# octavian-ganea/equidock_public

Hardware: NVIDIA H100
Metric: protein_pairs_per_sec_iegmn_fwd_kabsch (higher is better)
Workload: dtype f32

## Files before the change

### equidock_public_b200/csrc/node_mlp_tc.cu

```cuda
#include "tc_common.cuh"

namespace eqd {

#define NM_THREADS 256
#define NM_W5_SPLIT 34816
#define NM_W6_BASE 104448
#define NM_W6_SPLIT 8192
#define NM_W_BYTES 129024

struct NmConsts { float b5[64], ln_g[64], ln_b[64], b6[64]; };

#define NM_CHAINS 2
#define NM_SLOTS 3

struct NmSmem {
  unsigned char w[NM_W_BYTES];
  float stage[NM_CHAINS][NM_SLOTS][64 * 64];
  float c[256];
  unsigned long long w_bar;
};

#define NM_HLN_BYTES 512
static_assert(sizeof(NmSmem) + 128 + NM_HLN_BYTES <= 232448, "node MLP shared memory exceeds the sm_90 limit");

template <int P, bool HLN>
__global__ void __launch_bounds__(NM_CHAINS * 128, 1)
node_mlp_tc_kernel(int n_nodes, eqd_layer_params p, const __grid_constant__ NmConsts cst, const float* __restrict__ h_in,
                   const float* __restrict__ aggr, const float* __restrict__ mu, const float* __restrict__ h0,
                   float* __restrict__ h_out, eqd_layer_norms nm) {
  extern __shared__ __align__(128) unsigned char smem_raw[];
  NmSmem& S = *reinterpret_cast<NmSmem*>(smem_raw);
  float* hln = reinterpret_cast<float*>(smem_raw + sizeof(NmSmem));
  const int tid = threadIdx.x, wgi = tid >> 7, t = tid & 127, lane = t & 31;
  float (&ring)[NM_SLOTS][64 * 64] = S.stage[wgi];
  const int bar = 1 + wgi;
  const int ntiles = (n_nodes + 63) / 64, tstride = gridDim.x * NM_CHAINS, tile0 = blockIdx.x * NM_CHAINS + wgi;
  if (tid == 0) {
    mbar_init(&S.w_bar, 1);
    asm volatile("fence.mbarrier_init.release.cluster;" ::: "memory");
    mbar_expect_tx(&S.w_bar, NM_W_BYTES);
    bulk_g2s(S.w, p.w_node_tc, NM_W_BYTES, &S.w_bar);
  }
  for (int i = tid; i < 256; i += NM_CHAINS * 128) S.c[i] = reinterpret_cast<const float*>(&cst)[i];
  if (HLN && tid < 128) hln[tid] = tid < 64 ? nm.final_ln_g[tid] : nm.final_ln_b[tid - 64];
  __syncthreads();
  const unsigned w_saddr = smem_u32(S.w);
  const float slope = p.leaky_slope, sk = p.skip_weight_h, sk1 = 1.f - p.skip_weight_h;
  const int fr0 = (t >> 5) * 16 + (lane >> 2), fc = 2 * (lane & 3);

  auto issue = [&](int q) {
    const int tile = tile0 + (q >> 2) * tstride, pc = q & 3;
    if (tile < ntiles) {
      const float* src = pc == 0 ? h_in : pc == 1 ? aggr : pc == 2 ? mu : h0;
      stage_rows64(ring[q % NM_SLOTS], src, pc == 3 ? EQD_H0_PAD : EQD_HID, 0, (long)tile * 64, min(64, n_nodes - tile * 64), t);
    } else {
      cp_async_commit();
    }
  };
  int q = 0;
  for (int i = 0; i < NM_SLOTS - 1; ++i) issue(i);
  mbar_wait(&S.w_bar, 0);

  for (int tile = tile0; tile < ntiles; tile += tstride) {
    const int node0 = tile * 64, nvalid = min(64, n_nodes - node0);
    float2 x4[2];
#pragma unroll
    for (int hh = 0; hh < 2; ++hh) {
      const int row = fr0 + 8 * hh;
      x4[hh] = row < nvalid ? *reinterpret_cast<const float2*>(h0 + (long)(node0 + row) * EQD_H0_PAD + 64 + fc)
                            : make_float2(0.f, 0.f);
    }
    float acc[32], hs[32];
#pragma unroll
    for (int j = 0; j < 8; ++j) {
      const float2 bj = *reinterpret_cast<const float2*>(&S.c[8 * j + fc]);
#pragma unroll
      for (int hh = 0; hh < 2; ++hh) {
        acc[4 * j + 2 * hh] = bj.x;
        acc[4 * j + 2 * hh + 1] = bj.y;
      }
    }
#pragma unroll 1
    for (int pc = 0; pc < 4; ++pc, ++q) {
      cp_async_wait<NM_SLOTS - 2>();
      wg_barrier(bar);
      issue(q + NM_SLOTS - 1);
      float v[32];
      staged_rows_to_frag(ring[q % NM_SLOTS], t, v);
      if (pc == 0) {
#pragma unroll
        for (int i = 0; i < 32; ++i) hs[i] = v[i];
      }
      unsigned af[3][4][4];
      acc_to_a_split3<4, P>(v, af);
      float d[32];
      wg_gemm6_rs_issue<64, 4, 0, false, P>(d, af, [&](int sp, int kb) {
        return b_desc_ex(w_saddr + (4 * pc + kb) * 2048 + sp * NM_W5_SPLIT, 1024, 128); }, false);
      wg_mma_wait(d);
#pragma unroll
      for (int i = 0; i < 32; ++i) acc[i] = __fadd_rn(acc[i], d[i]);
    }
    {
      unsigned a4[3][1][4];
#pragma unroll
      for (int hh = 0; hh < 2; ++hh) split3_pair<P>(x4[hh].x, x4[hh].y, a4[0][0][hh], a4[1][0][hh], a4[2][0][hh]);
#pragma unroll
      for (int sp = 0; sp < 3; ++sp) a4[sp][0][2] = a4[sp][0][3] = 0u;
      float d[32];
      wg_gemm6_rs_issue<64, 1, 0, false, P>(d, a4, [&](int sp, int kb) {
        return b_desc_ex(w_saddr + 16 * 2048 + sp * NM_W5_SPLIT, 1024, 128); }, false);
      wg_mma_wait(d);
#pragma unroll
      for (int i = 0; i < 32; ++i) acc[i] = __fadd_rn(acc[i], d[i]);
    }
    unsigned af[3][4][4];
    {
      float (&v)[32] = acc;
#pragma unroll
      for (int i = 0; i < 32; ++i) v[i] = fmaxf(v[i], __fmul_rn(v[i], slope));
      float pv[32];
#pragma unroll
      for (int i = 0; i < 32; ++i) pv[i] = __shfl_xor_sync(0xffffffffu, v[i], 2);
      float msum[2], rstd[2];
#pragma unroll
      for (int h = 0; h < 2; ++h) {
        float mh[2], qh[2];
#pragma unroll
        for (int ch = 0; ch < 2; ++ch) {
          float s0 = 0.f, s1 = 0.f;
#pragma unroll
          for (int c4 = 0; c4 < 8; ++c4) {
            s0 = __fadd_rn(s0, chain_val(v, pv, h, ch, c4, 0));
            s1 = __fadd_rn(s1, chain_val(v, pv, h, ch, c4, 1));
          }
          const float sp = __fadd_rn(s0, s1);
          mh[ch] = __fmul_rn(__fadd_rn(sp, __shfl_xor_sync(0xffffffffu, sp, 1)), 1.f / 32.f);
          float q0 = 0.f, q1 = 0.f;
#pragma unroll
          for (int c4 = 0; c4 < 8; ++c4) {
            const float d0 = __fadd_rn(chain_val(v, pv, h, ch, c4, 0), -mh[ch]);
            const float d1 = __fadd_rn(chain_val(v, pv, h, ch, c4, 1), -mh[ch]);
            q0 = __fmaf_rn(d0, d0, q0);
            q1 = __fmaf_rn(d1, d1, q1);
          }
          const float qp = __fadd_rn(q0, q1);
          qh[ch] = __fadd_rn(qp, __shfl_xor_sync(0xffffffffu, qp, 1));
        }
        msum[h] = __fadd_rn(mh[0], mh[1]);
        const float dm = __fadd_rn(mh[0], -mh[1]);
        const float var = __fmaf_rn(__fmul_rn(dm, dm), 16.f, __fadd_rn(qh[0], qh[1]));
        rstd[h] = 1.f / sqrtf(__fmaf_rn(var, 1.f / 64.f, 1e-5f));
      }
#pragma unroll
      for (int j = 0; j < 8; ++j) {
        const float2 gj = *reinterpret_cast<const float2*>(&S.c[64 + 8 * j + fc]);
        const float2 bj = *reinterpret_cast<const float2*>(&S.c[128 + 8 * j + fc]);
#pragma unroll
        for (int h = 0; h < 2; ++h) {
          float& x0 = v[4 * j + 2 * h];
          float& x1 = v[4 * j + 2 * h + 1];
          x0 = __fmaf_rn(__fmul_rn(__fmaf_rn(msum[h], -0.5f, x0), rstd[h]), gj.x, bj.x);
          x1 = __fmaf_rn(__fmul_rn(__fmaf_rn(msum[h], -0.5f, x1), rstd[h]), gj.y, bj.y);
        }
      }
      acc_to_a_split3<4, P>(v, af);
    }
    {
      float d[32];
      wg_gemm6_rs_issue<64, 4, 0, false, P>(d, af, [&](int sp, int kb) {
        return b_desc_ex(w_saddr + NM_W6_BASE + sp * NM_W6_SPLIT + kb * 2048, 1024, 128); }, false);
      wg_mma_wait(d);
      if (HLN) {
#pragma unroll
        for (int j = 0; j < 8; ++j) {
          const float2 bj = *reinterpret_cast<const float2*>(&S.c[192 + 8 * j + fc]);
#pragma unroll
          for (int hh = 0; hh < 2; ++hh) {
            const int i = 4 * j + 2 * hh;
            d[i] = __fmaf_rn(__fadd_rn(d[i], bj.x), sk, __fmul_rn(hs[i], sk1));
            d[i + 1] = __fmaf_rn(__fadd_rn(d[i + 1], bj.y), sk, __fmul_rn(hs[i + 1], sk1));
          }
        }
        float mean[2], rstd[2];
        quad_ln_stats(d, mean, rstd);
        quad_ln_apply(d, mean, rstd, hln, hln + 64, fc);
#pragma unroll
        for (int hh = 0; hh < 2; ++hh) {
          const int row = fr0 + 8 * hh;
          if (row < nvalid) {
            float* o = h_out + (long)(node0 + row) * EQD_HID + fc;
#pragma unroll
            for (int j = 0; j < 8; ++j)
              *reinterpret_cast<float2*>(o + 8 * j) = make_float2(d[4 * j + 2 * hh], d[4 * j + 2 * hh + 1]);
          }
        }
      } else
#pragma unroll
      for (int hh = 0; hh < 2; ++hh) {
        const int row = fr0 + 8 * hh;
        if (row < nvalid) {
          float* o = h_out + (long)(node0 + row) * EQD_HID + fc;
#pragma unroll
          for (int j = 0; j < 8; ++j) {
            const float2 bj = *reinterpret_cast<const float2*>(&S.c[192 + 8 * j + fc]);
            const int i = 4 * j + 2 * hh;
            *reinterpret_cast<float2*>(o + 8 * j) =
                make_float2(__fmaf_rn(__fadd_rn(d[i], bj.x), sk, __fmul_rn(hs[i], sk1)),
                            __fmaf_rn(__fadd_rn(d[i + 1], bj.y), sk, __fmul_rn(hs[i + 1], sk1)));
          }
        }
      }
    }
  }
  cp_async_wait<0>();
}


#define NM0_W5_SPLIT 35840
#define NM0_W6_BASE 107520
#define NM0_W6_SPLIT 10240
#define NM0_W_BYTES 138240
#define NM0_A_SPLIT 20480
#define NM0_LD 84

struct Nm0Consts { float b5[80], ln_g[80], ln_b[80], b6[64]; };

struct Nm0Smem {
  unsigned char w[NM0_W_BYTES];
  unsigned char a[3 * NM0_A_SPLIT];
  float red[EQD_TM * 4];
  unsigned long long w_bar;
};

template <bool HLN>
__global__ void __launch_bounds__(NM_THREADS, 1)
node_mlp0_tc_kernel(int n_nodes, eqd_layer_params p, const __grid_constant__ Nm0Consts cst, const float* __restrict__ h0,
                    const float* __restrict__ aggr, const float* __restrict__ mu , float* __restrict__ h_out,
                    eqd_layer_norms nm) {
  extern __shared__ __align__(128) unsigned char smem_raw[];
  Nm0Smem& S = *reinterpret_cast<Nm0Smem*>(smem_raw);
  const int tid = threadIdx.x, q = tid, half = q >> 7, r = q & 127, wgi = tid >> 7;
  const int ntiles = (n_nodes + EQD_TM - 1) / EQD_TM;
  if (tid == 0) {
    mbar_init(&S.w_bar, 1);
    asm volatile("fence.mbarrier_init.release.cluster;" ::: "memory");
    mbar_expect_tx(&S.w_bar, NM0_W_BYTES);
    bulk_g2s(S.w, p.w_node_tc, NM0_W_BYTES, &S.w_bar);
  }
  __syncthreads();
  const unsigned w_saddr = smem_u32(S.w), a_saddr = smem_u32(S.a);
  float* const dtile = reinterpret_cast<float*>(S.a);
  auto a_desc = [&](int sp, int kb) { return a_desc_at<EQD_TM>(a_saddr, NM0_A_SPLIT, wgi, sp, kb); };
  mbar_wait(&S.w_bar, 0);
  const float slope = p.leaky_slope;
  float* red = S.red;

  for (int tile = blockIdx.x; tile < ntiles; tile += gridDim.x) {
    const int node = tile * EQD_TM + r;
    const bool valid = node < n_nodes;
    auto row32 = [&](const float* base, int ld, float (&v)[32]) {
      const float4* sp = reinterpret_cast<const float4*>(base + (long)node * ld + half * 32);
#pragma unroll
      for (int c4 = 0; c4 < 8; ++c4) {
        float4 t = valid ? sp[c4] : make_float4(0.f, 0.f, 0.f, 0.f);
        v[c4 * 4] = t.x; v[c4 * 4 + 1] = t.y; v[c4 * 4 + 2] = t.z; v[c4 * 4 + 3] = t.w;
      }
    };
    auto extra8 = [&](const float* base) {
      if (half == 0) {
        const float4* ep = reinterpret_cast<const float4*>(base + (long)node * EQD_H0_PAD + 64);
        float4 a = valid ? ep[0] : make_float4(0.f, 0.f, 0.f, 0.f), b = valid ? ep[1] : make_float4(0.f, 0.f, 0.f, 0.f);
        float t[8] = {a.x, a.y, a.z, a.w, b.x, b.y, b.z, b.w};
        store_extra8_split3<EQD_TM>(S.a, NM0_A_SPLIT, r, 64, t);
      }
    };
    float acc[32], accx[16];
#pragma unroll
    for (int c = 0; c < 32; ++c) acc[c] = cst.b5[half * 32 + c];
#pragma unroll
    for (int c = 0; c < 16; ++c) accx[c] = cst.b5[64 + c];
    auto piece = [&](int kb0, int nkb) {
      tc_fence_before();
      __syncthreads();
      {
        float d[40];
        wg_gemm6<80>(d, a_desc, [&](int sp, int kb) {
          return b_desc_ex(w_saddr + (kb0 + kb) * (80 * 32) + sp * NM0_W5_SPLIT, 80 * 16, 128); }, nkb, false);
        __syncthreads();
        wg_store_d<80>(dtile + wgi * 64 * NM0_LD, NM0_LD, d, tid & 127);
      }
      __syncthreads();
      const float* dr = dtile + r * NM0_LD;
#pragma unroll
      for (int c = 0; c < 32; ++c) acc[c] += dr[half * 32 + c];
      if (half == 0) {
#pragma unroll
        for (int c = 0; c < 16; ++c) accx[c] += dr[64 + c];
      }
      __syncthreads();
    };
    {
      float v[32];
      row32(h0, EQD_H0_PAD, v);
      store_half_split3<EQD_TM>(S.a, NM0_A_SPLIT, r, half * 32, v);
      extra8(h0);
      piece(0, 5);
      row32(aggr, EQD_HID, v);
      store_half_split3<EQD_TM>(S.a, NM0_A_SPLIT, r, half * 32, v);
      piece(5, 4);
      row32(mu, EQD_H0_PAD, v);
      store_half_split3<EQD_TM>(S.a, NM0_A_SPLIT, r, half * 32, v);
      extra8(mu);
      piece(9, 5);
    }
    {
      const int nh = half == 0 ? 37 : 32;
      float sum = 0.f;
#pragma unroll
      for (int c = 0; c < 32; ++c) {
        acc[c] = lrelu(acc[c], slope);
        sum += acc[c];
      }
      if (half == 0) {
#pragma unroll
        for (int c = 0; c < 5; ++c) {
          accx[c] = lrelu(accx[c], slope);
          sum += accx[c];
        }
      }
      const float mh = sum / (float)nh;
      float m2 = 0.f;
#pragma unroll
      for (int c = 0; c < 32; ++c) {
        float d = acc[c] - mh;
        m2 = fmaf(d, d, m2);
      }
      if (half == 0) {
#pragma unroll
        for (int c = 0; c < 5; ++c) {
          float d = accx[c] - mh;
          m2 = fmaf(d, d, m2);
        }
      }
      red[(r * 2 + half) * 2 + 0] = mh;
      red[(r * 2 + half) * 2 + 1] = m2;
      __syncthreads();
      const float m0 = red[r * 4 + 0], m1 = red[r * 4 + 2];
      const float mean = (37.f * m0 + 32.f * m1) * (1.f / 69.f);
      const float dm = m0 - m1;
      const float var = (red[r * 4 + 1] + red[r * 4 + 3] + dm * dm * (37.f * 32.f / 69.f)) * (1.f / 69.f);
      const float rstd = 1.f / sqrtf(var + 1e-5f);
#pragma unroll
      for (int c = 0; c < 32; ++c) acc[c] = (acc[c] - mean) * rstd * cst.ln_g[half * 32 + c] + cst.ln_b[half * 32 + c];
      store_half_split3<EQD_TM>(S.a, NM0_A_SPLIT, r, half * 32, acc);
      if (half == 0) {
        float t[8];
#pragma unroll
        for (int c = 0; c < 5; ++c) t[c] = (accx[c] - mean) * rstd * cst.ln_g[64 + c] + cst.ln_b[64 + c];
        t[5] = t[6] = t[7] = 0.f;
        store_extra8_split3<EQD_TM>(S.a, NM0_A_SPLIT, r, 64, t);
      }
    }
    tc_fence_before();
    __syncthreads();
    {
      float d[32];
      wg_gemm6<64>(d, a_desc, [&](int sp, int kb) {
        return b_desc_ex(w_saddr + NM0_W6_BASE + sp * NM0_W6_SPLIT + kb * 2048, 1024, 128); }, 5, false);
      __syncthreads();
      wg_store_d<64>(dtile + wgi * 64 * NM0_LD, NM0_LD, d, tid & 127);
    }
    __syncthreads();
    {
      float v[32];
      tile_ld32f(dtile, NM0_LD, r, half * 32, v);
#pragma unroll
      for (int c = 0; c < 32; ++c) v[c] += cst.b6[half * 32 + c];
      if (HLN) {
        float s = 0.f;
#pragma unroll
        for (int c = 0; c < 32; ++c) s += v[c];
        red[(r * 2 + half) * 2] = s;
        __syncthreads();
        const float mean = (red[r * 4] + red[r * 4 + 2]) * (1.f / 64.f);
        float q = 0.f;
#pragma unroll
        for (int c = 0; c < 32; ++c) {
          const float dv = v[c] - mean;
          q = fmaf(dv, dv, q);
        }
        red[(r * 2 + half) * 2 + 1] = q;
        __syncthreads();
        const float rstd = 1.f / sqrtf((red[r * 4 + 1] + red[r * 4 + 3]) * (1.f / 64.f) + 1e-5f);
#pragma unroll
        for (int c = 0; c < 32; ++c) v[c] = (v[c] - mean) * rstd * nm.final_ln_g[half * 32 + c] + nm.final_ln_b[half * 32 + c];
      }
      if (valid) {
        float4* o = reinterpret_cast<float4*>(h_out + (long)node * EQD_HID + half * 32);
#pragma unroll
        for (int c4 = 0; c4 < 8; ++c4) o[c4] = make_float4(v[c4 * 4], v[c4 * 4 + 1], v[c4 * 4 + 2], v[c4 * 4 + 3]);
      }
    }
    __syncthreads();
  }
}

template <int P, bool HLN>
static int launch_node_mlp_tc(const eqd_graph* g, const eqd_layer* p_l, const float* h_in, const float* aggr,
                              const float* mu, const float* h0, float* h_out, void* stream) {
  NmConsts cst;
  memcpy(&cst, p_l->consts.node, sizeof(cst));
  const int ntiles = (g->n_nodes + 63) / 64;
  const size_t smem = sizeof(NmSmem) + 128 + (HLN ? NM_HLN_BYTES : 0);
  EQD_SET_SMEM((node_mlp_tc_kernel<P, HLN>), smem);
  int grid = (ntiles + NM_CHAINS - 1) / NM_CHAINS;
  if (grid > EQD_SMS) grid = EQD_SMS;
  node_mlp_tc_kernel<P, HLN><<<grid, NM_CHAINS * 128, smem, (cudaStream_t)stream>>>(g->n_nodes, p_l->dev, cst, h_in, aggr,
                                                                                   mu, h0, h_out, p_l->norms);
  EQD_CUDA_LAUNCH_CHECK();
  return EQD_OK;
}

}

extern "C" int eqd_node_mlp_tc(const eqd_graph* g, const eqd_layer* p_l, const float* h_in, const float* aggr,
                               const float* mu, const float* h0, float* h_out, void* stream) {
  const eqd_layer_params* p = p_l ? &p_l->dev : nullptr;
  if (!g || !p || !h_in || !aggr || !mu || !h0 || !h_out) return EQD_ERR_BAD_ARG;
  if (p_l->dropout.p > 0.f) return EQD_ERR_UNSUPPORTED;
  if (p->dh != 64 || p->dhp != 64) return EQD_ERR_UNSUPPORTED;
  if (!(p->leaky_slope >= 0.f && p->leaky_slope <= 1.f)) return EQD_ERR_UNSUPPORTED;
  const int products = eqd_mma_products(p);
  if (!products) return EQD_ERR_UNSUPPORTED;
  if (!p->w_node_tc || (reinterpret_cast<uintptr_t>(p->w_node_tc) & 15)) return EQD_ERR_BAD_ARG;
  const int hln = eqd_final_ln(p_l);
  if (hln < 0) return EQD_ERR_BAD_ARG;
  if (g->n_nodes <= 0) return EQD_OK;
  if (hln)
    return products == 3 ? eqd::launch_node_mlp_tc<3, true>(g, p_l, h_in, aggr, mu, h0, h_out, stream)
                         : eqd::launch_node_mlp_tc<6, true>(g, p_l, h_in, aggr, mu, h0, h_out, stream);
  return products == 3 ? eqd::launch_node_mlp_tc<3, false>(g, p_l, h_in, aggr, mu, h0, h_out, stream)
                       : eqd::launch_node_mlp_tc<6, false>(g, p_l, h_in, aggr, mu, h0, h_out, stream);
}

extern "C" int eqd_node_mlp_tc0(const eqd_graph* g, const eqd_layer* p_l, const float* h0, const float* aggr,
                                const float* mu, float* h_out, void* stream) {
  const eqd_layer_params* p = p_l ? &p_l->dev : nullptr;
  if (!g || !p || !h0 || !aggr || !mu || !h_out) return EQD_ERR_BAD_ARG;
  if (p_l->dropout.p > 0.f) return EQD_ERR_UNSUPPORTED;
  if (p->dh != 69 || p->dhp != 72 || !eqd_mma_products(p)) return EQD_ERR_UNSUPPORTED;
  if (!(p->leaky_slope >= 0.f && p->leaky_slope <= 1.f)) return EQD_ERR_UNSUPPORTED;
  if (!p->w_node_tc || (reinterpret_cast<uintptr_t>(p->w_node_tc) & 15)) return EQD_ERR_BAD_ARG;
  const int hln = eqd_final_ln(p_l);
  if (hln < 0) return EQD_ERR_BAD_ARG;
  if (g->n_nodes <= 0) return EQD_OK;
  eqd::Nm0Consts cst;
  memcpy(&cst, p_l->consts.node, sizeof(cst));
  int ntiles = (g->n_nodes + EQD_TM - 1) / EQD_TM;
  size_t smem = sizeof(eqd::Nm0Smem) + 128;
  int grid = ntiles < EQD_SMS ? ntiles : EQD_SMS;
  if (hln) {
    EQD_SET_SMEM((eqd::node_mlp0_tc_kernel<true>), smem);
    eqd::node_mlp0_tc_kernel<true><<<grid, NM_THREADS, smem, (cudaStream_t)stream>>>(g->n_nodes, *p, cst, h0, aggr, mu, h_out,
                                                                                    p_l->norms);
  } else {
    EQD_SET_SMEM((eqd::node_mlp0_tc_kernel<false>), smem);
    eqd::node_mlp0_tc_kernel<false><<<grid, NM_THREADS, smem, (cudaStream_t)stream>>>(g->n_nodes, *p, cst, h0, aggr, mu,
                                                                                     h_out, p_l->norms);
  }
  EQD_CUDA_LAUNCH_CHECK();
  return EQD_OK;
}

extern "C" int eqd_attention_tc0(const eqd_graph*, const float*, const void*, const float*, float*, void*);

extern "C" int eqd_node_stage_tc0(const eqd_graph* g, const eqd_layer* p_l, const eqd_layer* p_next_l,
                                  const float* h0, const float* proj, const float* aggr, void* kv, const float* x5,
                                  float* mu, float* h_out, float* proj_next, void* stream) {
  const eqd_layer_params* p = p_l ? &p_l->dev : nullptr;
  const eqd_layer_params* p_next = p_next_l ? &p_next_l->dev : nullptr;
  if (!g || !p || !kv || !mu || !x5) return EQD_ERR_BAD_ARG;
  if (p_next && !proj_next) return EQD_ERR_BAD_ARG;
  if (!eqd_mma_products(p)) return EQD_ERR_UNSUPPORTED;
  int rc = eqd_attention_tc0(g, proj, kv, x5, mu, stream);
  if (rc) return rc;
  rc = eqd_node_mlp_tc0(g, p_l, h0, aggr, mu, h_out, stream);
  if (rc) return rc;
  if (p_next) rc = eqd_project_tc(g, p_next_l, h_out, proj_next, kv, stream);
  return rc;
}

extern "C" int eqd_project_tc(const eqd_graph*, const eqd_layer*, const float*, float*, void*, void*);
int eqd_attention_tc_products(const eqd_graph*, const float*, const void*, float*, int, void*);


extern "C" int eqd_node_stage_tc(const eqd_graph* g, const eqd_layer* p_l, const eqd_layer* p_next_l,
                                 const float* h_in, const float* h0, const float* proj, const float* aggr, void* kv,
                                 float* mu, float* h_out, float* proj_next, void* stream) {
  const eqd_layer_params* p = p_l ? &p_l->dev : nullptr;
  const eqd_layer_params* p_next = p_next_l ? &p_next_l->dev : nullptr;
  if (!g || !p || !kv || !mu) return EQD_ERR_BAD_ARG;
  if (p_next && !proj_next) return EQD_ERR_BAD_ARG;
  const int products = eqd_mma_products(p);
  if (!products) return EQD_ERR_UNSUPPORTED;
  int rc = eqd_attention_tc_products(g, proj, kv, mu, products, stream);
  if (rc) return rc;
  rc = eqd_node_mlp_tc(g, p_l, h_in, aggr, mu, h0, h_out, stream);
  if (rc) return rc;
  if (p_next) rc = eqd_project_tc(g, p_next_l, h_out, proj_next, kv, stream);
  return rc;
}
```

### equidock_public_b200/csrc/proj_tc.cu

```cuda
#include "tc_common.cuh"

namespace eqd {

#define PJ_LD 68

template <bool L0>
struct PjCfg {
  static constexpr int R = L0 ? 64 : 128;
  static constexpr int THREADS = 2 * R;
  static constexpr int KB = L0 ? 5 : 4;
  static constexpr int GROUP_BYTES = 64 * KB * 16 * 2 * 3;
  static constexpr int SPLIT_BYTES = 64 * KB * 16 * 2;
  static constexpr int X_SPLIT_BYTES = 16 * KB * 16 * 2;
  static constexpr int W_BYTES = 5 * GROUP_BYTES + (L0 ? 3 * X_SPLIT_BYTES : 0);
  static constexpr int A_SPLIT_BYTES = R * KB * 32;
  static constexpr int NGROUPS = L0 ? 6 : 5;
};

struct PjConsts { float b[336]; };

template <bool L0>
struct PjSmem {
  unsigned char w[PjCfg<L0>::W_BYTES];
  unsigned char a[3 * PjCfg<L0>::A_SPLIT_BYTES];
  float d[PjCfg<L0>::R * PJ_LD];
  unsigned long long w_bar;
};

__device__ __forceinline__ void store_kv_blocks(unsigned char* __restrict__ kv, long split_stride, int node, int half,
                                                const float (&v)[32]) {
  unsigned p0[16], p1[16], p2[16];
#pragma unroll
  for (int c = 0; c < 16; ++c) split3_pair(v[2 * c], v[2 * c + 1], p0[c], p1[c], p2[c]);
  unsigned char* base = kv + (long)(node >> 3) * 1024 + (node & 7) * 16 + half * 512;
#pragma unroll
  for (int j = 0; j < 4; ++j) {
    *reinterpret_cast<uint4*>(base + j * 128) = make_uint4(p0[4 * j], p0[4 * j + 1], p0[4 * j + 2], p0[4 * j + 3]);
    *reinterpret_cast<uint4*>(base + split_stride + j * 128) = make_uint4(p1[4 * j], p1[4 * j + 1], p1[4 * j + 2], p1[4 * j + 3]);
    *reinterpret_cast<uint4*>(base + 2 * split_stride + j * 128) = make_uint4(p2[4 * j], p2[4 * j + 1], p2[4 * j + 2], p2[4 * j + 3]);
  }
}

template <bool L0>
__global__ void __launch_bounds__(PjCfg<L0>::THREADS, 1)
project_tc_kernel(int n_nodes, eqd_layer_params p, const __grid_constant__ PjConsts cst, const float* __restrict__ h, int ldh,
                  float* __restrict__ proj, int pw, unsigned char* __restrict__ kv, long kv_split_stride, float* __restrict__ x5) {
  using C = PjCfg<L0>;
  constexpr int R = C::R;
  extern __shared__ __align__(128) unsigned char smem_raw[];
  PjSmem<L0>& S = *reinterpret_cast<PjSmem<L0>*>(smem_raw);
  const int tid = threadIdx.x, half = tid / R, r = tid % R, warp = tid >> 5, wgi = tid >> 7;
  const int ntiles = (n_nodes + R - 1) / R;
  if (tid == 0) {
    mbar_init(&S.w_bar, 1);
    asm volatile("fence.mbarrier_init.release.cluster;" ::: "memory");
    mbar_expect_tx(&S.w_bar, C::W_BYTES);
    bulk_g2s(S.w, p.w_proj_tc, C::W_BYTES, &S.w_bar);
  }
  __syncthreads();
  const unsigned w_saddr = smem_u32(S.w), a_saddr = smem_u32(S.a);
  auto a_desc = [&](int s, int kb) { return a_desc_at<R>(a_saddr, C::A_SPLIT_BYTES, wgi, s, kb); };
  float* dslab = S.d + wgi * 64 * PJ_LD;
  mbar_wait(&S.w_bar, 0);
  const float slope = p.leaky_slope;
  const int lane = tid & 31, wrow0 = (warp * 32) % R;

  for (int tile = blockIdx.x; tile < ntiles; tile += gridDim.x) {
    const int node0 = tile * R;
    const int node = node0 + r;
    const bool valid = node < n_nodes;
    {
      float v[32];
      const float4* hp = reinterpret_cast<const float4*>(h + (long)node * ldh + half * 32);
#pragma unroll
      for (int c4 = 0; c4 < 8; ++c4) {
        float4 t = valid ? hp[c4] : make_float4(0.f, 0.f, 0.f, 0.f);
        v[c4 * 4] = t.x; v[c4 * 4 + 1] = t.y; v[c4 * 4 + 2] = t.z; v[c4 * 4 + 3] = t.w;
      }
      if (L0 && half == 0) {
        const float4* ep = reinterpret_cast<const float4*>(h + (long)node * ldh + 64);
        float4 a = valid ? ep[0] : make_float4(0.f, 0.f, 0.f, 0.f), b = valid ? ep[1] : make_float4(0.f, 0.f, 0.f, 0.f);
        float t[8] = {a.x, a.y, a.z, a.w, b.x, b.y, b.z, b.w};
        store_extra8_split3<R>(S.a, C::A_SPLIT_BYTES, r, 64, t);
      }
      store_half_split3<R>(S.a, C::A_SPLIT_BYTES, r, half * 32, v);
    }
    tc_fence_before();
    __syncthreads();
#pragma unroll 1
    for (int grp = 0; grp < C::NGROUPS; ++grp) {
      if (L0 && grp == 5) {
        float d[8];
        wg_gemm6<16>(d, a_desc, [&](int s, int kb) {
          return b_desc_ex(w_saddr + 5 * C::GROUP_BYTES + s * C::X_SPLIT_BYTES + kb * 512, 256, 128); }, C::KB, false);
        wg_store_d<16>(dslab, PJ_LD, d, tid & 127);
        __syncthreads();
        if (half == 0 && valid) {
          float e[16];
#pragma unroll
          for (int c = 0; c < 16; ++c) {
            const bool act = (c < 4) || c == 8 || (c >= 10 && c < 15);
            const float x = S.d[r * PJ_LD + c];
            e[c] = act ? lrelu(x, slope) : x;
          }
          float4* o = reinterpret_cast<float4*>(x5 + (long)node * 16);
#pragma unroll
          for (int c4 = 0; c4 < 4; ++c4) o[c4] = make_float4(e[c4 * 4], e[c4 * 4 + 1], e[c4 * 4 + 2], e[c4 * 4 + 3]);
        }
        continue;
      }
      {
        float d[32];
        wg_gemm6<64>(d, a_desc, [&](int s, int kb) {
          return b_desc_ex(w_saddr + grp * C::GROUP_BYTES + s * C::SPLIT_BYTES + kb * 2048, 1024, 128); }, C::KB, false);
        wg_store_d<64>(dslab, PJ_LD, d, tid & 127);
      }
      __syncthreads();
      float v[32];
      tile_ld32f(S.d, PJ_LD, r, half * 32, v);
      const bool act = (grp == 2 || grp == 3);
#pragma unroll
      for (int c = 0; c < 32; ++c) {
        float t = v[c] + cst.b[grp * 64 + half * 32 + c];
        v[c] = act ? lrelu(t, slope) : t;
      }
      if (grp < 3 || kv == nullptr) {
        if (L0) {
          if (valid) {
            float4* o = reinterpret_cast<float4*>(proj + (long)node * pw + grp * 64 + half * 32);
#pragma unroll
            for (int c4 = 0; c4 < 8; ++c4) o[c4] = make_float4(v[c4 * 4], v[c4 * 4 + 1], v[c4 * 4 + 2], v[c4 * 4 + 3]);
          }
        } else {
          float* sc = S.d + r * PJ_LD + half * 32;
#pragma unroll
          for (int c4 = 0; c4 < 8; ++c4)
            *reinterpret_cast<float4*>(sc + c4 * 4) = make_float4(v[c4 * 4], v[c4 * 4 + 1], v[c4 * 4 + 2], v[c4 * 4 + 3]);
          __syncwarp();
          float* o = proj + (long)(node0 + wrow0) * pw + grp * 64 + half * 32 + (lane & 7) * 4;
#pragma unroll
          for (int i = 0; i < 8; ++i) {
            const int row = i * 4 + (lane >> 3);
            float4 t = *reinterpret_cast<const float4*>(S.d + (wrow0 + row) * PJ_LD + half * 32 + (lane & 7) * 4);
            if (node0 + wrow0 + row < n_nodes) *reinterpret_cast<float4*>(o + (long)row * pw) = t;
          }
        }
      }
      if (valid && grp >= 3 && kv != nullptr)
        store_kv_blocks(kv + (long)(grp - 3) * 3 * kv_split_stride, kv_split_stride, node, half, v);
      __syncthreads();
    }
    __syncthreads();
  }
}

#define PJ_CHAINS 2
#define PJ64_W_BYTES (5 * PjCfg<false>::GROUP_BYTES)
#define PJ_OUT_LD 72

struct __align__(128) PjChainSmem {
  float hs[64 * 64];
  float out[64 * PJ_OUT_LD];
};
struct Pj64Smem {
  unsigned char w[PJ64_W_BYTES];
  PjChainSmem ch[PJ_CHAINS];
  float b[320];
  unsigned long long w_bar;
};

template <int P>
__global__ void __launch_bounds__(PJ_CHAINS * 128, 1)
project64_tc_kernel(int n_nodes, eqd_layer_params p, const __grid_constant__ PjConsts cst, const float* __restrict__ h,
                    float* __restrict__ proj, unsigned char* __restrict__ kv, long kv_split_stride) {
  extern __shared__ __align__(128) unsigned char smem_raw[];
  Pj64Smem& S = *reinterpret_cast<Pj64Smem*>(smem_raw);
  const int tid = threadIdx.x, wgi = tid >> 7, t = tid & 127, lane = t & 31;
  PjChainSmem& W = S.ch[wgi];
  const int bar = 1 + wgi;
  const int ntiles = (n_nodes + 63) / 64, tstride = gridDim.x * PJ_CHAINS;
  if (tid == 0) {
    mbar_init(&S.w_bar, 1);
    asm volatile("fence.mbarrier_init.release.cluster;" ::: "memory");
    mbar_expect_tx(&S.w_bar, PJ64_W_BYTES);
    bulk_g2s(S.w, p.w_proj_tc, PJ64_W_BYTES, &S.w_bar);
  }
  for (int i = tid; i < 320; i += PJ_CHAINS * 128) S.b[i] = cst.b[i];
  __syncthreads();
  const unsigned w_saddr = smem_u32(S.w);
  const float slope = p.leaky_slope;
  const int fr0 = (t >> 5) * 16 + (lane >> 2), fc = 2 * (lane & 3);
  auto stage_h = [&](int tile) { stage_rows64(W.hs, h, EQD_HID, 0, (long)tile * 64, min(64, n_nodes - tile * 64), t); };
  int tile = blockIdx.x * PJ_CHAINS + wgi;
  if (tile < ntiles) stage_h(tile);
  mbar_wait(&S.w_bar, 0);

  for (; tile < ntiles; tile += tstride) {
    const int node0 = tile * 64, nvalid = min(64, n_nodes - node0);
    cp_async_wait<0>();
    wg_barrier(bar);
    unsigned af[3][4][4];
    staged_rows_to_a_split3<P>(W.hs, t, af);
    wg_barrier(bar);
    if (tile + tstride < ntiles) stage_h(tile + tstride);
    auto group = [&](int grp) {
      return [&, grp](int s, int kb) { return b_desc_ex(w_saddr + grp * PjCfg<false>::GROUP_BYTES + s * PjCfg<false>::SPLIT_BYTES + kb * 2048, 1024, 128); };
    };
    float acc[2][32];
    wg_gemm6_rs_issue<64, 4, 0, false, P>(acc[0], af, group(0), false);
#pragma unroll
    for (int grp = 0; grp < 5; ++grp) {
      float (&d)[32] = acc[grp & 1];
      if (grp + 1 < 5) {
        wg_gemm6_rs_issue<64, 4, 0, false, P>(acc[(grp + 1) & 1], af, group(grp + 1), false);
        wg_mma_wait<1>(d);
      } else {
        wg_mma_wait(d);
      }
      const bool act = (grp == 2 || grp == 3);
#pragma unroll
      for (int j = 0; j < 8; ++j) {
        const float2 bj = *reinterpret_cast<const float2*>(&S.b[grp * 64 + 8 * j + fc]);
#pragma unroll
        for (int hh = 0; hh < 2; ++hh) {
          float& x0 = d[4 * j + 2 * hh];
          float& x1 = d[4 * j + 2 * hh + 1];
          x0 = x0 + bj.x;
          x1 = x1 + bj.y;
          if (act) {
            x0 = lrelu(x0, slope);
            x1 = lrelu(x1, slope);
          }
        }
      }
      if (grp < 3 || kv == nullptr) {
#pragma unroll
        for (int j = 0; j < 8; ++j)
#pragma unroll
          for (int hh = 0; hh < 2; ++hh)
            *reinterpret_cast<float2*>(W.out + (fr0 + 8 * hh) * PJ_OUT_LD + 8 * j + fc) =
                make_float2(d[4 * j + 2 * hh], d[4 * j + 2 * hh + 1]);
        wg_barrier(bar);
#pragma unroll
        for (int i = 0; i < 8; ++i) {
          const int row = i * 8 + (t >> 4), c4 = t & 15;
          if (row < nvalid)
            *reinterpret_cast<float4*>(proj + (long)(node0 + row) * 320 + grp * 64 + 4 * c4) =
                *reinterpret_cast<const float4*>(W.out + row * PJ_OUT_LD + 4 * c4);
        }
        wg_barrier(bar);
      } else {
        unsigned char* base = kv + (long)(grp - 3) * 3 * kv_split_stride;
#pragma unroll
        for (int hh = 0; hh < 2; ++hh) {
          const int row = fr0 + 8 * hh, node = node0 + row;
          if (row < nvalid) {
            unsigned char* nb = base + (long)(node >> 3) * 1024 + (node & 7) * 16 + fc * 2;
#pragma unroll
            for (int j = 0; j < 8; ++j) {
              unsigned w0, w1, w2;
              split3_pair(d[4 * j + 2 * hh], d[4 * j + 2 * hh + 1], w0, w1, w2);
              *reinterpret_cast<unsigned*>(nb + j * 128) = w0;
              *reinterpret_cast<unsigned*>(nb + kv_split_stride + j * 128) = w1;
              *reinterpret_cast<unsigned*>(nb + 2 * kv_split_stride + j * 128) = w2;
            }
          }
        }
      }
    }
  }
  cp_async_wait<0>();
}

__global__ void kv_blocks_kernel(int n_nodes, const float* __restrict__ proj, int pw, int koff, int voff,
                                 unsigned char* __restrict__ kv, long kv_split_stride) {
  int idx = blockIdx.x * blockDim.x + threadIdx.x;
  int node = idx >> 2, which = (idx >> 1) & 1, half = idx & 1;
  if (node >= n_nodes) return;
  const float4* src = reinterpret_cast<const float4*>(proj + (long)node * pw + (which ? voff : koff) + half * 32);
  float v[32];
#pragma unroll
  for (int c4 = 0; c4 < 8; ++c4) {
    float4 t = src[c4];
    v[c4 * 4] = t.x; v[c4 * 4 + 1] = t.y; v[c4 * 4 + 2] = t.z; v[c4 * 4 + 3] = t.w;
  }
  store_kv_blocks(kv + (long)which * 3 * kv_split_stride, kv_split_stride, node, half, v);
}

}

extern "C" size_t eqd_kv_blocks_bytes(int32_t n_nodes) {
  return (size_t)6 * ((size_t)(n_nodes + 7) / 8 + 8) * 1024;
}

template <bool L0>
static int launch_project_tc(const eqd_graph* g, const eqd_layer* p_l, const float* h, int ldh, float* proj, int pw,
                             void* kv, float* x5, void* stream) {
  const eqd_layer_params* p = &p_l->dev;
  if (!(p->leaky_slope >= 0.f && p->leaky_slope <= 1.f)) return EQD_ERR_UNSUPPORTED;
  if (!p->w_proj_tc || (reinterpret_cast<uintptr_t>(p->w_proj_tc) & 15)) return EQD_ERR_BAD_ARG;
  if (g->n_nodes <= 0) return EQD_OK;
  eqd::PjConsts cst;
  memset(&cst, 0, sizeof(cst));
  memcpy(&cst, p_l->consts.proj_bias, 320 * sizeof(float));
  int ntiles = (g->n_nodes + eqd::PjCfg<L0>::R - 1) / eqd::PjCfg<L0>::R;
  size_t smem = sizeof(eqd::PjSmem<L0>) + 128;
  EQD_SET_SMEM((eqd::project_tc_kernel<L0>), smem);
  int grid = ntiles < EQD_SMS ? ntiles : EQD_SMS;
  long split_stride = (long)((g->n_nodes + 7) / 8 + 8) * 1024;
  eqd::project_tc_kernel<L0><<<grid, eqd::PjCfg<L0>::THREADS, smem, (cudaStream_t)stream>>>(
      g->n_nodes, *p, cst, h, ldh, proj, pw, reinterpret_cast<unsigned char*>(kv), split_stride, x5);
  EQD_CUDA_LAUNCH_CHECK();
  return EQD_OK;
}

template <int P>
static int launch_project64_tc(const eqd_graph* g, const eqd_layer* p_l, const float* h, float* proj, void* kv,
                               void* stream) {
  eqd::PjConsts cst;
  memset(&cst, 0, sizeof(cst));
  memcpy(&cst, p_l->consts.proj_bias, 320 * sizeof(float));
  const int ntiles = (g->n_nodes + 63) / 64;
  const size_t smem = sizeof(eqd::Pj64Smem) + 128;
  EQD_SET_SMEM(eqd::project64_tc_kernel<P>, smem);
  int grid = (ntiles + PJ_CHAINS - 1) / PJ_CHAINS;
  if (grid > EQD_SMS) grid = EQD_SMS;
  const long split_stride = (long)((g->n_nodes + 7) / 8 + 8) * 1024;
  eqd::project64_tc_kernel<P><<<grid, PJ_CHAINS * 128, smem, (cudaStream_t)stream>>>(
      g->n_nodes, p_l->dev, cst, h, proj, reinterpret_cast<unsigned char*>(kv), split_stride);
  EQD_CUDA_LAUNCH_CHECK();
  return EQD_OK;
}

extern "C" int eqd_project_tc(const eqd_graph* g, const eqd_layer* p_l, const float* h, float* proj, void* kv,
                              void* stream) {
  const eqd_layer_params* p = p_l ? &p_l->dev : nullptr;
  if (!g || !p || !h || !proj) return EQD_ERR_BAD_ARG;
  if (p->dh != 64 || p->dhp != 64) return EQD_ERR_UNSUPPORTED;
  if (!(p->leaky_slope >= 0.f && p->leaky_slope <= 1.f)) return EQD_ERR_UNSUPPORTED;
  const int products = eqd_mma_products(p);
  if (!products) return EQD_ERR_UNSUPPORTED;
  if (!p->w_proj_tc || (reinterpret_cast<uintptr_t>(p->w_proj_tc) & 15)) return EQD_ERR_BAD_ARG;
  if (g->n_nodes <= 0) return EQD_OK;
  return products == 3 ? launch_project64_tc<3>(g, p_l, h, proj, kv, stream)
                       : launch_project64_tc<6>(g, p_l, h, proj, kv, stream);
}

extern "C" int eqd_project_tc0(const eqd_graph* g, const eqd_layer* p_l, const float* h0, float* proj, void* kv,
                               float* x5, void* stream) {
  const eqd_layer_params* p = p_l ? &p_l->dev : nullptr;
  if (!g || !p || !h0 || !proj || !kv || !x5) return EQD_ERR_BAD_ARG;
  if (p->dh != 69 || p->dhp != 72 || !eqd_mma_products(p)) return EQD_ERR_UNSUPPORTED;
  return launch_project_tc<true>(g, p_l, h0, EQD_H0_PAD, proj, 128 + 3 * 72, kv, x5, stream);
}

extern "C" int eqd_kv_blocks(const eqd_graph* g, const float* proj, int32_t pw, int32_t koff, int32_t voff, void* kv,
                             void* stream) {
  if (!g || !proj || !kv) return EQD_ERR_BAD_ARG;
  if (g->n_nodes <= 0) return EQD_OK;
  long split_stride = (long)((g->n_nodes + 7) / 8 + 8) * 1024;
  int total = g->n_nodes * 4;
  eqd::kv_blocks_kernel<<<(total + 255) / 256, 256, 0, (cudaStream_t)stream>>>(g->n_nodes, proj, pw, koff, voff,
                                                                                reinterpret_cast<unsigned char*>(kv), split_stride);
  EQD_CUDA_LAUNCH_CHECK();
  return EQD_OK;
}
```

### equidock_public_b200/csrc/tc_common.cuh

```cuda
#pragma once
#include "common.cuh"

namespace eqd {

__device__ __forceinline__ unsigned smem_u32(const void* p) { return (unsigned)__cvta_generic_to_shared(p); }

__device__ __forceinline__ void mbar_init(unsigned long long* bar, int count) {
  asm volatile("mbarrier.init.shared::cta.b64 [%0], %1;" ::"r"(smem_u32(bar)), "r"(count));
}
__device__ __forceinline__ void mbar_wait(unsigned long long* bar, unsigned parity) {
  unsigned addr = smem_u32(bar);
  unsigned done = 0;
  while (!done) {
    asm volatile(
        "{\n\t.reg .pred p;\n\t"
        "mbarrier.try_wait.parity.shared::cta.b64 p, [%1], %2;\n\t"
        "selp.u32 %0, 1, 0, p;\n\t}"
        : "=r"(done) : "r"(addr), "r"(parity) : "memory");
  }
}
__device__ __forceinline__ void mbar_expect_tx(unsigned long long* bar, unsigned bytes) {
  asm volatile("mbarrier.arrive.expect_tx.shared::cta.b64 _, [%0], %1;" ::"r"(smem_u32(bar)), "r"(bytes) : "memory");
}
__device__ __forceinline__ void bulk_g2s(void* dst, const void* src, unsigned bytes, unsigned long long* bar) {
  asm volatile("cp.async.bulk.shared::cluster.global.mbarrier::complete_tx::bytes [%0], [%1], %2, [%3];" ::"r"(smem_u32(dst)),
               "l"(src), "r"(bytes), "r"(smem_u32(bar)) : "memory");
}
__device__ __forceinline__ void cp_async8(void* dst, const void* src) {
  asm volatile("cp.async.ca.shared.global [%0], [%1], 8;" ::"r"(smem_u32(dst)), "l"(src));
}
__device__ __forceinline__ void cp_async4(void* dst, const void* src) {
  asm volatile("cp.async.ca.shared.global [%0], [%1], 4;" ::"r"(smem_u32(dst)), "l"(src));
}
__device__ __forceinline__ void tc_fence_before() { asm volatile("fence.proxy.async.shared::cta;" ::: "memory"); }

__device__ __forceinline__ unsigned long long b_desc_ex(unsigned saddr, unsigned lbo, unsigned sbo) {
  return (unsigned long long)((saddr >> 4) & 0x3FFF) | ((unsigned long long)((lbo >> 4) & 0x3FFF) << 16) |
         ((unsigned long long)((sbo >> 4) & 0x3FFF) << 32);
}

template <int N, int TB>
struct Wgmma;
template <int TB>
struct Wgmma<16, TB> {
  static __device__ __forceinline__ void mma(float (&d)[8], unsigned long long a, unsigned long long b, int scale_d) {
    asm volatile(
        "{\n\t.reg .pred p;\n\tsetp.ne.b32 p, %10, 0;\n\t"
        "wgmma.mma_async.sync.aligned.m64n16k16.f32.bf16.bf16 {%0, %1, %2, %3, %4, %5, %6, %7}, %8, %9, p, 1, 1, 0, %11;\n\t}"
        : "+f"(d[0]), "+f"(d[1]), "+f"(d[2]), "+f"(d[3]), "+f"(d[4]), "+f"(d[5]), "+f"(d[6]), "+f"(d[7])
        : "l"(a), "l"(b), "r"(scale_d), "n"(TB));
  }
};
template <int TB>
struct Wgmma<64, TB> {
  static __device__ __forceinline__ void mma(float (&d)[32], unsigned long long a, unsigned long long b, int scale_d) {
    asm volatile(
        "{\n\t.reg .pred p;\n\tsetp.ne.b32 p, %34, 0;\n\t"
        "wgmma.mma_async.sync.aligned.m64n64k16.f32.bf16.bf16 {%0, %1, %2, %3, %4, %5, %6, %7, %8, %9, %10, %11, %12, %13, %14, %15, %16, %17, %18, %19, %20, %21, %22, %23, %24, %25, %26, %27, %28, %29, %30, %31}, %32, %33, p, 1, 1, 0, %35;\n\t}"
        : "+f"(d[0]), "+f"(d[1]), "+f"(d[2]), "+f"(d[3]), "+f"(d[4]), "+f"(d[5]), "+f"(d[6]), "+f"(d[7]), "+f"(d[8]), "+f"(d[9]), "+f"(d[10]), "+f"(d[11]), "+f"(d[12]), "+f"(d[13]), "+f"(d[14]), "+f"(d[15]), "+f"(d[16]), "+f"(d[17]), "+f"(d[18]), "+f"(d[19]), "+f"(d[20]), "+f"(d[21]), "+f"(d[22]), "+f"(d[23]), "+f"(d[24]), "+f"(d[25]), "+f"(d[26]), "+f"(d[27]), "+f"(d[28]), "+f"(d[29]), "+f"(d[30]), "+f"(d[31])
        : "l"(a), "l"(b), "r"(scale_d), "n"(TB));
  }
};
template <int TB>
struct Wgmma<80, TB> {
  static __device__ __forceinline__ void mma(float (&d)[40], unsigned long long a, unsigned long long b, int scale_d) {
    asm volatile(
        "{\n\t.reg .pred p;\n\tsetp.ne.b32 p, %42, 0;\n\t"
        "wgmma.mma_async.sync.aligned.m64n80k16.f32.bf16.bf16 {%0, %1, %2, %3, %4, %5, %6, %7, %8, %9, %10, %11, %12, %13, %14, %15, %16, %17, %18, %19, %20, %21, %22, %23, %24, %25, %26, %27, %28, %29, %30, %31, %32, %33, %34, %35, %36, %37, %38, %39}, %40, %41, p, 1, 1, 0, %43;\n\t}"
        : "+f"(d[0]), "+f"(d[1]), "+f"(d[2]), "+f"(d[3]), "+f"(d[4]), "+f"(d[5]), "+f"(d[6]), "+f"(d[7]), "+f"(d[8]), "+f"(d[9]), "+f"(d[10]), "+f"(d[11]), "+f"(d[12]), "+f"(d[13]), "+f"(d[14]), "+f"(d[15]), "+f"(d[16]), "+f"(d[17]), "+f"(d[18]), "+f"(d[19]), "+f"(d[20]), "+f"(d[21]), "+f"(d[22]), "+f"(d[23]), "+f"(d[24]), "+f"(d[25]), "+f"(d[26]), "+f"(d[27]), "+f"(d[28]), "+f"(d[29]), "+f"(d[30]), "+f"(d[31]), "+f"(d[32]), "+f"(d[33]), "+f"(d[34]), "+f"(d[35]), "+f"(d[36]), "+f"(d[37]), "+f"(d[38]), "+f"(d[39])
        : "l"(a), "l"(b), "r"(scale_d), "n"(TB));
  }
};

template <int N, int TB>
struct WgmmaRS;
template <int TB>
struct WgmmaRS<64, TB> {
  static __device__ __forceinline__ void mma(float (&d)[32], const unsigned (&a)[4], unsigned long long b, int scale_d) {
    asm volatile(
        "{\n\t.reg .pred p;\n\tsetp.ne.b32 p, %37, 0;\n\t"
        "wgmma.mma_async.sync.aligned.m64n64k16.f32.bf16.bf16 {%0, %1, %2, %3, %4, %5, %6, %7, %8, %9, %10, %11, %12, %13, %14, %15, %16, %17, %18, %19, %20, %21, %22, %23, %24, %25, %26, %27, %28, %29, %30, %31}, {%32, %33, %34, %35}, %36, p, 1, 1, %38;\n\t}"
        : "+f"(d[0]), "+f"(d[1]), "+f"(d[2]), "+f"(d[3]), "+f"(d[4]), "+f"(d[5]), "+f"(d[6]), "+f"(d[7]), "+f"(d[8]), "+f"(d[9]), "+f"(d[10]), "+f"(d[11]), "+f"(d[12]), "+f"(d[13]), "+f"(d[14]), "+f"(d[15]), "+f"(d[16]), "+f"(d[17]), "+f"(d[18]), "+f"(d[19]), "+f"(d[20]), "+f"(d[21]), "+f"(d[22]), "+f"(d[23]), "+f"(d[24]), "+f"(d[25]), "+f"(d[26]), "+f"(d[27]), "+f"(d[28]), "+f"(d[29]), "+f"(d[30]), "+f"(d[31])
        : "r"(a[0]), "r"(a[1]), "r"(a[2]), "r"(a[3]), "l"(b), "r"(scale_d), "n"(TB));
  }
};

template <int N, int TB = 0, int P = 6, class AD, class BD>
__device__ __forceinline__ void wg_gemm6_issue(float (&d)[N / 2], AD a_desc, BD b_desc, int kblocks, bool accumulate,
                                               bool hi_only = false) {
  static_assert(P == 6 || P == 3, "bf16x6 or bf16x3");
  const int pa[6] = {2, 0, 1, 1, 0, 0}, pb[6] = {0, 2, 1, 0, 1, 0};
  asm volatile("wgmma.fence.sync.aligned;" ::: "memory");
  int scale_d = accumulate ? 1 : 0;
#pragma unroll
  for (int pr = hi_only ? 5 : 6 - P; pr < 6; ++pr)
    for (int kb = 0; kb < kblocks; ++kb) {
      Wgmma<N, TB>::mma(d, a_desc(pa[pr], kb), b_desc(pb[pr], kb), scale_d);
      scale_d = 1;
    }
  asm volatile("wgmma.commit_group.sync.aligned;" ::: "memory");
}
template <int PENDING = 0, int M>
__device__ __forceinline__ void wg_mma_wait(float (&d)[M]) {
  asm volatile("wgmma.wait_group.sync.aligned %0;" ::"n"(PENDING) : "memory");
#pragma unroll
  for (int i = 0; i < M; ++i) asm volatile("" : "+f"(d[i])::"memory");
}
template <int N, int TB = 0, int P = 6, class AD, class BD>
__device__ __forceinline__ void wg_gemm6(float (&d)[N / 2], AD a_desc, BD b_desc, int kblocks, bool accumulate,
                                         bool hi_only = false) {
  wg_gemm6_issue<N, TB, P>(d, a_desc, b_desc, kblocks, accumulate, hi_only);
  asm volatile("wgmma.wait_group.sync.aligned 0;" ::: "memory");
}
template <int N, int KB, int TB = 0, bool HI_ONLY = false, int P = 6, class BD>
__device__ __forceinline__ void wg_gemm6_rs_issue(float (&d)[N / 2], const unsigned (&a)[3][KB][4], BD b_desc, bool accumulate) {
  static_assert(P == 6 || P == 3, "bf16x6 or bf16x3");
  constexpr int pa[6] = {2, 0, 1, 1, 0, 0}, pb[6] = {0, 2, 1, 0, 1, 0};
  asm volatile("wgmma.fence.sync.aligned;" ::: "memory");
  int scale_d = accumulate ? 1 : 0;
#pragma unroll
  for (int pr = HI_ONLY ? 5 : 6 - P; pr < 6; ++pr)
#pragma unroll
    for (int kb = 0; kb < KB; ++kb) {
      WgmmaRS<N, TB>::mma(d, a[pa[pr]][kb], b_desc(pb[pr], kb), scale_d);
      scale_d = 1;
    }
  asm volatile("wgmma.commit_group.sync.aligned;" ::: "memory");
}

template <int R>
__device__ __forceinline__ unsigned long long a_desc_at(unsigned a_saddr, unsigned split_bytes, int wgi, int s, int kb) {
  return b_desc_ex(a_saddr + s * split_bytes + kb * (32 * R) + wgi * 1024, 16 * R, 128);
}
template <int R, int P = 6>
__device__ __forceinline__ void a_store8(unsigned char* a, unsigned split_bytes, int row, int c, const unsigned* p0,
                                         const unsigned* p1, const unsigned* p2) {
  unsigned char* base = a + (c >> 4) * (32 * R) + ((c >> 3) & 1) * (16 * R) + (row >> 3) * 128 + (row & 7) * 16;
  *reinterpret_cast<uint4*>(base) = make_uint4(p0[0], p0[1], p0[2], p0[3]);
  *reinterpret_cast<uint4*>(base + split_bytes) = make_uint4(p1[0], p1[1], p1[2], p1[3]);
  if constexpr (P == 6) *reinterpret_cast<uint4*>(base + 2 * split_bytes) = make_uint4(p2[0], p2[1], p2[2], p2[3]);
}

template <int N>
__device__ __forceinline__ void wg_store_d(float* tile, int ld, const float (&d)[N / 2], int t) {
  const int row = (t >> 5) * 16 + ((t & 31) >> 2), col = 2 * (t & 3);
#pragma unroll
  for (int j = 0; j < N / 8; ++j) {
    *reinterpret_cast<float2*>(tile + row * ld + 8 * j + col) = make_float2(d[4 * j], d[4 * j + 1]);
    *reinterpret_cast<float2*>(tile + (row + 8) * ld + 8 * j + col) = make_float2(d[4 * j + 2], d[4 * j + 3]);
  }
}

__device__ __forceinline__ unsigned cvt_bf16x2(float hi, float lo) {
  unsigned d;
  asm("cvt.rn.bf16x2.f32 %0, %1, %2;" : "=r"(d) : "f"(hi), "f"(lo));
  return d;
}
template <int P = 6>
__device__ __forceinline__ void split3_pair(float v0, float v1, unsigned& p0, unsigned& p1, unsigned& p2) {
  p0 = cvt_bf16x2(v1, v0);
  const float r0 = v0 - __uint_as_float(p0 << 16), r1 = v1 - __uint_as_float(p0 & 0xFFFF0000u);
  p1 = cvt_bf16x2(r1, r0);
  if constexpr (P == 6) p2 = cvt_bf16x2(r1 - __uint_as_float(p1 & 0xFFFF0000u), r0 - __uint_as_float(p1 << 16));
}
template <int R>
__device__ __forceinline__ void store_half_split3(unsigned char* a, unsigned split_bytes, int row, int c0, const float (&v)[32]) {
  unsigned p0[16], p1[16], p2[16];
#pragma unroll
  for (int c = 0; c < 16; ++c) split3_pair(v[2 * c], v[2 * c + 1], p0[c], p1[c], p2[c]);
#pragma unroll
  for (int j = 0; j < 4; ++j) a_store8<R>(a, split_bytes, row, c0 + 8 * j, p0 + 4 * j, p1 + 4 * j, p2 + 4 * j);
}
template <int R>
__device__ __forceinline__ void store_extra8_split3(unsigned char* a, unsigned split_bytes, int row, int c0, const float (&t)[8]) {
  unsigned p0[8], p1[8], p2[8];
#pragma unroll
  for (int c = 0; c < 4; ++c) split3_pair(t[2 * c], t[2 * c + 1], p0[c], p1[c], p2[c]);
#pragma unroll
  for (int c = 4; c < 8; ++c) p0[c] = p1[c] = p2[c] = 0u;
  a_store8<R>(a, split_bytes, row, c0, p0, p1, p2);
  a_store8<R>(a, split_bytes, row, c0 + 8, p0 + 4, p1 + 4, p2 + 4);
}
template <int KB, int P = 6>
__device__ __forceinline__ void acc_to_a_split3(const float (&v)[8 * KB], unsigned (&a)[3][KB][4]) {
#pragma unroll
  for (int kb = 0; kb < KB; ++kb)
#pragma unroll
    for (int i = 0; i < 4; ++i) split3_pair<P>(v[8 * kb + 2 * i], v[8 * kb + 2 * i + 1], a[0][kb][i], a[1][kb][i], a[2][kb][i]);
}
__device__ __forceinline__ int stage_swz(int row) { return (row & 3) << 1; }
__device__ __forceinline__ void stage_rows64(float* rows, const float* src, int ld, int col0, long row0, int nvalid, int t) {
#pragma unroll
  for (int i = 0; i < 8; ++i) {
    const int idx = i * 128 + t, row = idx >> 4, k4 = idx & 15;
    const bool ok = row < nvalid;
    cp_async16(rows + row * 64 + ((k4 ^ stage_swz(row)) << 2), src + (row0 + (ok ? row : 0)) * ld + col0 + 4 * k4, ok);
  }
  cp_async_commit();
}
template <int P = 6>
__device__ __forceinline__ void staged_rows_to_a_split3(const float* rows, int t, unsigned (&a)[3][4][4]) {
  const int g = (t >> 5) * 16 + ((t & 31) >> 2), c = t & 3;
#pragma unroll
  for (int kb = 0; kb < 4; ++kb)
#pragma unroll
    for (int i = 0; i < 4; ++i) {
      const int row = g + 8 * (i & 1), k4 = 4 * kb + 2 * (i >> 1) + (c >> 1);
      const float2 v = *reinterpret_cast<const float2*>(rows + row * 64 + ((k4 ^ stage_swz(row)) << 2) + 2 * (c & 1));
      split3_pair<P>(v.x, v.y, a[0][kb][i], a[1][kb][i], a[2][kb][i]);
    }
}
__device__ __forceinline__ void staged_rows_to_frag(const float* rows, int t, float (&v)[32]) {
  const int g = (t >> 5) * 16 + ((t & 31) >> 2), c = t & 3;
#pragma unroll
  for (int kb = 0; kb < 4; ++kb)
#pragma unroll
    for (int i = 0; i < 4; ++i) {
      const int row = g + 8 * (i & 1), k4 = 4 * kb + 2 * (i >> 1) + (c >> 1);
      const float2 x = *reinterpret_cast<const float2*>(rows + row * 64 + ((k4 ^ stage_swz(row)) << 2) + 2 * (c & 1));
      v[8 * kb + 2 * i] = x.x;
      v[8 * kb + 2 * i + 1] = x.y;
    }
}
__device__ __forceinline__ float chain_val(const float (&v)[32], const float (&pv)[32], int h, int ch, int c4, int e) {
  const int i = 4 * (4 * ch + (c4 >> 1)) + 2 * h + e;
  const bool own = ((c4 & 1) == 0) == ((threadIdx.x & 2) == 0);
  return own ? v[i] : pv[i];
}
__device__ __forceinline__ void wg_barrier(int id) { asm volatile("bar.sync %0, 128;" ::"r"(id) : "memory"); }
__device__ __forceinline__ bool wg_barrier_and(int id, bool pred) {
  unsigned all;
  asm volatile(
      "{\n\t.reg .pred p, q;\n\tsetp.ne.u32 p, %1, 0;\n\t"
      "bar.red.and.pred q, %2, 128, p;\n\tselp.u32 %0, 1, 0, q;\n\t}"
      : "=r"(all) : "r"((unsigned)pred), "r"(id) : "memory");
  return all != 0;
}
__device__ __forceinline__ void tile_ld32f(const float* tile, int ld, int row, int c0, float (&v)[32]) {
  const float4* s = reinterpret_cast<const float4*>(tile + row * ld + c0);
#pragma unroll
  for (int c4 = 0; c4 < 8; ++c4) {
    float4 t = s[c4];
    v[c4 * 4] = t.x; v[c4 * 4 + 1] = t.y; v[c4 * 4 + 2] = t.z; v[c4 * 4 + 3] = t.w;
  }
}

__device__ __forceinline__ void quad_ln_stats(const float (&v)[32], float (&mean)[2], float (&rstd)[2]) {
  float pv[32];
#pragma unroll
  for (int i = 0; i < 32; ++i) pv[i] = __shfl_xor_sync(0xffffffffu, v[i], 2);
#pragma unroll
  for (int h = 0; h < 2; ++h) {
    float mh[2], qh[2];
#pragma unroll
    for (int ch = 0; ch < 2; ++ch) {
      float s0 = 0.f, s1 = 0.f;
#pragma unroll
      for (int c4 = 0; c4 < 8; ++c4) {
        s0 = __fadd_rn(s0, chain_val(v, pv, h, ch, c4, 0));
        s1 = __fadd_rn(s1, chain_val(v, pv, h, ch, c4, 1));
      }
      const float sp = s0 + s1;
      mh[ch] = (sp + __shfl_xor_sync(0xffffffffu, sp, 1)) * (1.f / 32.f);
      float q0 = 0.f, q1 = 0.f;
#pragma unroll
      for (int c4 = 0; c4 < 8; ++c4) {
        const float d0 = __fadd_rn(chain_val(v, pv, h, ch, c4, 0), -mh[ch]);
        const float d1 = __fadd_rn(chain_val(v, pv, h, ch, c4, 1), -mh[ch]);
        q0 = fmaf(d0, d0, q0);
        q1 = fmaf(d1, d1, q1);
      }
      const float qp = q0 + q1;
      qh[ch] = qp + __shfl_xor_sync(0xffffffffu, qp, 1);
    }
    const float m0 = mh[0], m1 = mh[1];
    mean[h] = 0.5f * (m0 + m1);
    const float dm = m0 - m1;
    const float var = (qh[0] + qh[1] + dm * dm * 16.f) * (1.f / 64.f);
    rstd[h] = 1.f / sqrtf(var + 1e-5f);
  }
}

__device__ __forceinline__ void quad_ln_apply(float (&v)[32], const float (&mean)[2], const float (&rstd)[2],
                                              const float* ln_g, const float* ln_b, int fc) {
#pragma unroll
  for (int j = 0; j < 8; ++j) {
    const float2 gj = *reinterpret_cast<const float2*>(&ln_g[8 * j + fc]);
    const float2 bj = *reinterpret_cast<const float2*>(&ln_b[8 * j + fc]);
#pragma unroll
    for (int h = 0; h < 2; ++h) {
      float& x0 = v[4 * j + 2 * h];
      float& x1 = v[4 * j + 2 * h + 1];
      x0 = fmaf(__fmul_rn(__fadd_rn(x0, -mean[h]), rstd[h]), gj.x, bj.x);
      x1 = fmaf(__fmul_rn(__fadd_rn(x1, -mean[h]), rstd[h]), gj.y, bj.y);
    }
  }
}

}
```

Baseline: 42770.

## Restructure layer-0 node MLP into per-warpgroup pipelined chains with register-A wgmma

Rewrites the layer-0 node MLP kernel so each 128-thread warpgroup independently processes 64-row tiles. Input pieces are staged through a double-buffered cp.async ring, and A fragments are built in registers for register-source wgmma instead of being written into split smem tiles. Block-wide __syncthreads are replaced by named per-warpgroup barriers, and bias and LayerNorm constants move to shared memory. The project-0 launch also switches to a dedicated chained kernel. This aims to overlap global loads with MMA and cut barrier and smem round-trip costs, at the price of more register pressure and more complex code.

```diff
diff --git a/equidock_public_b200/csrc/node_mlp_tc.cu b/equidock_public_b200/csrc/node_mlp_tc.cu
--- a/equidock_public_b200/csrc/node_mlp_tc.cu
+++ b/equidock_public_b200/csrc/node_mlp_tc.cu
@@ -2,7 +2,6 @@
 
 namespace eqd {
 
-#define NM_THREADS 256
 #define NM_W5_SPLIT 34816
 #define NM_W6_BASE 104448
 #define NM_W6_SPLIT 8192
@@ -220,189 +219,239 @@
 #define NM0_W6_BASE 107520
 #define NM0_W6_SPLIT 10240
 #define NM0_W_BYTES 138240
-#define NM0_A_SPLIT 20480
-#define NM0_LD 84
+#define NM0_LD 80
 
 struct Nm0Consts { float b5[80], ln_g[80], ln_b[80], b6[64]; };
 
 struct Nm0Smem {
   unsigned char w[NM0_W_BYTES];
-  unsigned char a[3 * NM0_A_SPLIT];
-  float red[EQD_TM * 4];
+  float stage[NM_CHAINS][2][64 * NM0_LD];
+  float red[NM_CHAINS][64 * 4];
+  float c[304];
   unsigned long long w_bar;
 };
+static_assert(sizeof(Nm0Smem) + 128 + NM_HLN_BYTES <= 232448, "layer-0 node MLP shared memory exceeds the sm_90 limit");
+
+__device__ __forceinline__ int nm0_ix(int row, int col) {
+  return row * NM0_LD + (col < 64 ? ((((col >> 2) ^ (row & 7)) << 2) | (col & 3)) : col);
+}
 
 template <bool HLN>
-__global__ void __launch_bounds__(NM_THREADS, 1)
+__global__ void __launch_bounds__(NM_CHAINS * 128, 1)
 node_mlp0_tc_kernel(int n_nodes, eqd_layer_params p, const __grid_constant__ Nm0Consts cst, const float* __restrict__ h0,
                     const float* __restrict__ aggr, const float* __restrict__ mu , float* __restrict__ h_out,
                     eqd_layer_norms nm) {
   extern __shared__ __align__(128) unsigned char smem_raw[];
   Nm0Smem& S = *reinterpret_cast<Nm0Smem*>(smem_raw);
-  const int tid = threadIdx.x, q = tid, half = q >> 7, r = q & 127, wgi = tid >> 7;
-  const int ntiles = (n_nodes + EQD_TM - 1) / EQD_TM;
+  float* hln = reinterpret_cast<float*>(smem_raw + sizeof(Nm0Smem));
+  const int tid = threadIdx.x, wgi = tid >> 7, t = tid & 127, lane = t & 31;
+  float (&ring)[2][64 * NM0_LD] = S.stage[wgi];
+  float* const red = S.red[wgi];
+  const int bar = 1 + wgi;
+  const int ntiles = (n_nodes + 63) / 64, tstride = gridDim.x * NM_CHAINS, tile0 = blockIdx.x * NM_CHAINS + wgi;
   if (tid == 0) {
     mbar_init(&S.w_bar, 1);
     asm volatile("fence.mbarrier_init.release.cluster;" ::: "memory");
     mbar_expect_tx(&S.w_bar, NM0_W_BYTES);
     bulk_g2s(S.w, p.w_node_tc, NM0_W_BYTES, &S.w_bar);
   }
+  for (int i = tid; i < 304; i += NM_CHAINS * 128) S.c[i] = reinterpret_cast<const float*>(&cst)[i];
+  if (HLN && tid < 128) hln[tid] = tid < 64 ? nm.final_ln_g[tid] : nm.final_ln_b[tid - 64];
   __syncthreads();
-  const unsigned w_saddr = smem_u32(S.w), a_saddr = smem_u32(S.a);
-  float* const dtile = reinterpret_cast<float*>(S.a);
-  auto a_desc = [&](int sp, int kb) { return a_desc_at<EQD_TM>(a_saddr, NM0_A_SPLIT, wgi, sp, kb); };
+  const unsigned w_saddr = smem_u32(S.w);
+  const float slope = p.leaky_slope;
+  const int fr0 = (t >> 5) * 16 + (lane >> 2), fc = 2 * (lane & 3);
+  const int lr = t & 63, lh = t >> 6;
+  const float* const b5 = S.c;
+  const float* const ln_g = S.c + 80;
+  const float* const ln_b = S.c + 160;
+  const float* const b6 = S.c + 240;
+
+  auto issue = [&](int q) {
+    const int tile = tile0 + (q / 3) * tstride, pc = q % 3;
+    if (tile < ntiles) {
+      const float* src = pc == 0 ? h0 : pc == 1 ? aggr : mu;
+      stage_rows64(ring[q & 1], src, pc == 1 ? EQD_HID : EQD_H0_PAD, 0, (long)tile * 64, min(64, n_nodes - tile * 64), t);
+    } else {
+      cp_async_commit();
+    }
+  };
+  int q = 0;
+  issue(0);
   mbar_wait(&S.w_bar, 0);
-  const float slope = p.leaky_slope;
-  float* red = S.red;
-
-  for (int tile = blockIdx.x; tile < ntiles; tile += gridDim.x) {
-    const int node = tile * EQD_TM + r;
-    const bool valid = node < n_nodes;
-    auto row32 = [&](const float* base, int ld, float (&v)[32]) {
-      const float4* sp = reinterpret_cast<const float4*>(base + (long)node * ld + half * 32);
+
+  for (int tile = tile0; tile < ntiles; tile += tstride) {
+    const int node0 = tile * 64, nvalid = min(64, n_nodes - node0);
+    float acc[40];
+#pragma unroll
+    for (int j = 0; j < 10; ++j) {
+      const float2 bj = *reinterpret_cast<const float2*>(&b5[8 * j + fc]);
+#pragma unroll
+      for (int hh = 0; hh < 2; ++hh) {
+        acc[4 * j + 2 * hh] = bj.x;
+        acc[4 * j + 2 * hh + 1] = bj.y;
+      }
+    }
+    auto piece = [&](auto kbc, int kb0, const float* extra) {
+      constexpr int KB = decltype(kbc)::value;
+      unsigned af[3][KB][4];
+      if constexpr (KB == 5) extra8_to_a_split3<5>(extra, EQD_H0_PAD, 64, node0, nvalid, t, 4, af);
+      cp_async_wait<0>();
+      wg_barrier(bar);
+      issue(q + 1);
+      {
+        unsigned a4[3][4][4];
+        staged_rows_to_a_split3(ring[q & 1], t, a4);
+#pragma unroll
+        for (int sp = 0; sp < 3; ++sp)
+#pragma unroll
+          for (int kb = 0; kb < 4; ++kb)
+#pragma unroll
+            for (int i = 0; i < 4; ++i) af[sp][kb][i] = a4[sp][kb][i];
+      }
+      float d[40];
+      wg_gemm6_rs_issue<80, KB>(d, af, [&](int sp, int kb) {
+        return b_desc_ex(w_saddr + (kb0 + kb) * (80 * 32) + sp * NM0_W5_SPLIT, 80 * 16, 128); }, false);
+      wg_mma_wait(d);
+#pragma unroll
+      for (int i = 0; i < 40; ++i) acc[i] = __fadd_rn(acc[i], d[i]);
+      ++q;
+    };
+#pragma unroll 1
+    for (int pc = 0; pc < 3; ++pc) {
+      if (pc == 1) piece(std::integral_constant<int, 4>{}, 5, nullptr);
+      else piece(std::integral_constant<int, 5>{}, pc == 0 ? 0 : 9, pc == 0 ? h0 : mu);
+    }
+    float* const tl = ring[(q - 1) & 1];
+#pragma unroll
+    for (int i = 0; i < 40; ++i) acc[i] = fmaxf(acc[i], __fmul_rn(acc[i], slope));
+    wg_barrier(bar);
+#pragma unroll
+    for (int j = 0; j < 9; ++j)
+#pragma unroll
+      for (int hh = 0; hh < 2; ++hh)
+        *reinterpret_cast<float2*>(tl + nm0_ix(fr0 + 8 * hh, 8 * j + fc)) = make_float2(acc[4 * j + 2 * hh], acc[4 * j + 2 * hh + 1]);
+    wg_barrier(bar);
+    {
+      float x[37];
 #pragma unroll
       for (int c4 = 0; c4 < 8; ++c4) {
-        float4 t = valid ? sp[c4] : make_float4(0.f, 0.f, 0.f, 0.f);
-        v[c4 * 4] = t.x; v[c4 * 4 + 1] = t.y; v[c4 * 4 + 2] = t.z; v[c4 * 4 + 3] = t.w;
-      }
-    };
-    auto extra8 = [&](const float* base) {
-      if (half == 0) {
-        const float4* ep = reinterpret_cast<const float4*>(base + (long)node * EQD_H0_PAD + 64);
-        float4 a = valid ? ep[0] : make_float4(0.f, 0.f, 0.f, 0.f), b = valid ? ep[1] : make_float4(0.f, 0.f, 0.f, 0.f);
-        float t[8] = {a.x, a.y, a.z, a.w, b.x, b.y, b.z, b.w};
-        store_extra8_split3<EQD_TM>(S.a, NM0_A_SPLIT, r, 64, t);
-      }
-    };
-    float acc[32], accx[16];
-#pragma unroll
-    for (int c = 0; c < 32; ++c) acc[c] = cst.b5[half * 32 + c];
-#pragma unroll
-    for (int c = 0; c < 16; ++c) accx[c] = cst.b5[64 + c];
-    auto piece = [&](int kb0, int nkb) {
-      tc_fence_before();
-      __syncthreads();
+        const float4 v4 = *reinterpret_cast<const float4*>(tl + nm0_ix(lr, lh * 32 + 4 * c4));
+        x[4 * c4] = v4.x; x[4 * c4 + 1] = v4.y; x[4 * c4 + 2] = v4.z; x[4 * c4 + 3] = v4.w;
+      }
+      const int nx = lh == 0 ? 37 : 32;
+#pragma unroll
+      for (int c = 32; c < 37; ++c) x[c] = lh == 0 ? tl[nm0_ix(lr, 32 + c)] : 0.f;
+      float sum = 0.f;
+#pragma unroll
+      for (int c = 0; c < 37; ++c)
+        if (c < nx) sum = __fadd_rn(sum, x[c]);
+      const float mh = __fdiv_rn(sum, (float)nx);
+      float m2 = 0.f;
+#pragma unroll
+      for (int c = 0; c < 37; ++c)
+        if (c < nx) {
+          const float dv = __fadd_rn(x[c], -mh);
+          m2 = __fmaf_rn(dv, dv, m2);
+        }
+      red[lr * 4 + lh * 2] = mh;
+      red[lr * 4 + lh * 2 + 1] = m2;
+    }
+    wg_barrier(bar);
+    unsigned af[3][5][4];
+    {
+      float s37[2], rstd[2];
+#pragma unroll
+      for (int hh = 0; hh < 2; ++hh) {
+        const float4 rs = *reinterpret_cast<const float4*>(red + (fr0 + 8 * hh) * 4);
+        s37[hh] = __fmaf_rn(rs.x, 37.f, __fmul_rn(rs.z, 32.f));
+        const float dm = __fadd_rn(rs.x, -rs.z);
+        const float var = __fmaf_rn(__fmul_rn(dm, dm), 37.f * 32.f / 69.f, __fadd_rn(rs.y, rs.w));
+        rstd[hh] = 1.f / sqrtf(__fmaf_rn(var, 1.f / 69.f, 1e-5f));
+      }
+#pragma unroll
+      for (int j = 0; j < 10; ++j)
+#pragma unroll
+        for (int e = 0; e < 2; ++e) {
+          const int col = 8 * j + fc + e;
+          const float g = col < 69 ? ln_g[col] : 0.f, b = col < 69 ? ln_b[col] : 0.f;
+#pragma unroll
+          for (int hh = 0; hh < 2; ++hh) {
+            float& v = acc[4 * j + 2 * hh + e];
+            v = col < 69 ? __fmaf_rn(__fmul_rn(__fmaf_rn(s37[hh], -(1.f / 69.f), v), rstd[hh]), g, b) : 0.f;
+          }
+        }
+      acc_to_a_split3<5>(acc, af);
+    }
+    float d[32];
+    wg_gemm6_rs_issue<64, 5>(d, af, [&](int sp, int kb) {
+      return b_desc_ex(w_saddr + NM0_W6_BASE + sp * NM0_W6_SPLIT + kb * 2048, 1024, 128); }, false);
+    wg_mma_wait(d);
+#pragma unroll
+    for (int j = 0; j < 8; ++j) {
+      const float2 bj = *reinterpret_cast<const float2*>(&b6[8 * j + fc]);
+#pragma unroll
+      for (int hh = 0; hh < 2; ++hh) {
+        d[4 * j + 2 * hh] = __fadd_rn(d[4 * j + 2 * hh], bj.x);
+        d[4 * j + 2 * hh + 1] = __fadd_rn(d[4 * j + 2 * hh + 1], bj.y);
+      }
+    }
+    if (HLN) {
+#pragma unroll
+      for (int j = 0; j < 8; ++j)
+#pragma unroll
+        for (int hh = 0; hh < 2; ++hh)
+          *reinterpret_cast<float2*>(tl + nm0_ix(fr0 + 8 * hh, 8 * j + fc)) = make_float2(d[4 * j + 2 * hh], d[4 * j + 2 * hh + 1]);
+      wg_barrier(bar);
+      float x[32];
+#pragma unroll
+      for (int c4 = 0; c4 < 8; ++c4) {
+        const float4 v4 = *reinterpret_cast<const float4*>(tl + nm0_ix(lr, lh * 32 + 4 * c4));
+        x[4 * c4] = v4.x; x[4 * c4 + 1] = v4.y; x[4 * c4 + 2] = v4.z; x[4 * c4 + 3] = v4.w;
+      }
+      float sum = 0.f;
+#pragma unroll
+      for (int c = 0; c < 32; ++c) sum = __fadd_rn(sum, x[c]);
+      red[lr * 4 + lh * 2] = sum;
+      wg_barrier(bar);
       {
-        float d[40];
-        wg_gemm6<80>(d, a_desc, [&](int sp, int kb) {
-          return b_desc_ex(w_saddr + (kb0 + kb) * (80 * 32) + sp * NM0_W5_SPLIT, 80 * 16, 128); }, nkb, false);
-        __syncthreads();
-        wg_store_d<80>(dtile + wgi * 64 * NM0_LD, NM0_LD, d, tid & 127);
-      }
-      __syncthreads();
-      const float* dr = dtile + r * NM0_LD;
-#pragma unroll
-      for (int c = 0; c < 32; ++c) acc[c] += dr[half * 32 + c];
-      if (half == 0) {
-#pragma unroll
-        for (int c = 0; c < 16; ++c) accx[c] += dr[64 + c];
-      }
-      __syncthreads();
-    };
-    {
-      float v[32];
-      row32(h0, EQD_H0_PAD, v);
-      store_half_split3<EQD_TM>(S.a, NM0_A_SPLIT, r, half * 32, v);
-      extra8(h0);
-      piece(0, 5);
-      row32(aggr, EQD_HID, v);
-      store_half_split3<EQD_TM>(S.a, NM0_A_SPLIT, r, half * 32, v);
-      piece(5, 4);
-      row32(mu, EQD_H0_PAD, v);
-      store_half_split3<EQD_TM>(S.a, NM0_A_SPLIT, r, half * 32, v);
-      extra8(mu);
-      piece(9, 5);
-    }
-    {
-      const int nh = half == 0 ? 37 : 32;
-      float sum = 0.f;
-#pragma unroll
-      for (int c = 0; c < 32; ++c) {
-        acc[c] = lrelu(acc[c], slope);
-        sum += acc[c];
-      }
-      if (half == 0) {
-#pragma unroll
-        for (int c = 0; c < 5; ++c) {
-          accx[c] = lrelu(accx[c], slope);
-          sum += accx[c];
-        }
-      }
-      const float mh = sum / (float)nh;
-      float m2 = 0.f;
-#pragma unroll
-      for (int c = 0; c < 32; ++c) {
-        float d = acc[c] - mh;
-        m2 = fmaf(d, d, m2);
-      }
-      if (half == 0) {
-#pragma unroll
-        for (int c = 0; c < 5; ++c) {
-          float d = accx[c] - mh;
-          m2 = fmaf(d, d, m2);
-        }
-      }
-      red[(r * 2 + half) * 2 + 0] = mh;
-      red[(r * 2 + half) * 2 + 1] = m2;
-      __syncthreads();
-      const float m0 = red[r * 4 + 0], m1 = red[r * 4 + 2];
-      const float mean = (37.f * m0 + 32.f * m1) * (1.f / 69.f);
-      const float dm = m0 - m1;
-      const float var = (red[r * 4 + 1] + red[r * 4 + 3] + dm * dm * (37.f * 32.f / 69.f)) * (1.f / 69.f);
-      const float rstd = 1.f / sqrtf(var + 1e-5f);
-#pragma unroll
-      for (int c = 0; c < 32; ++c) acc[c] = (acc[c] - mean) * rstd * cst.ln_g[half * 32 + c] + cst.ln_b[half * 32 + c];
-      store_half_split3<EQD_TM>(S.a, NM0_A_SPLIT, r, half * 32, acc);
-      if (half == 0) {
-        float t[8];
-#pragma unroll
-        for (int c = 0; c < 5; ++c) t[c] = (accx[c] - mean) * rstd * cst.ln_g[64 + c] + cst.ln_b[64 + c];
-        t[5] = t[6] = t[7] = 0.f;
-        store_extra8_split3<EQD_TM>(S.a, NM0_A_SPLIT, r, 64, t);
-      }
-    }
-    tc_fence_before();
-    __syncthreads();
-    {
-      float d[32];
-      wg_gemm6<64>(d, a_desc, [&](int sp, int kb) {
-        return b_desc_ex(w_saddr + NM0_W6_BASE + sp * NM0_W6_SPLIT + kb * 2048, 1024, 128); }, 5, false);
-      __syncthreads();
-      wg_store_d<64>(dtile + wgi * 64 * NM0_LD, NM0_LD, d, tid & 127);
-    }
-    __syncthreads();
-    {
-      float v[32];
-      tile_ld32f(dtile, NM0_LD, r, half * 32, v);
-#pragma unroll
-      for (int c = 0; c < 32; ++c) v[c] += cst.b6[half * 32 + c];
-      if (HLN) {
-        float s = 0.f;
-#pragma unroll
-        for (int c = 0; c < 32; ++c) s += v[c];
-        red[(r * 2 + half) * 2] = s;
-        __syncthreads();
-        const float mean = (red[r * 4] + red[r * 4 + 2]) * (1.f / 64.f);
-        float q = 0.f;
+        const float mean = __fmul_rn(__fadd_rn(red[lr * 4], red[lr * 4 + 2]), 1.f / 64.f);
+        float qs = 0.f;
 #pragma unroll
         for (int c = 0; c < 32; ++c) {
-          const float dv = v[c] - mean;
-          q = fmaf(dv, dv, q);
-        }
-        red[(r * 2 + half) * 2 + 1] = q;
-        __syncthreads();
-        const float rstd = 1.f / sqrtf((red[r * 4 + 1] + red[r * 4 + 3]) * (1.f / 64.f) + 1e-5f);
-#pragma unroll
-        for (int c = 0; c < 32; ++c) v[c] = (v[c] - mean) * rstd * nm.final_ln_g[half * 32 + c] + nm.final_ln_b[half * 32 + c];
-      }
-      if (valid) {
-        float4* o = reinterpret_cast<float4*>(h_out + (long)node * EQD_HID + half * 32);
-#pragma unroll
-        for (int c4 = 0; c4 < 8; ++c4) o[c4] = make_float4(v[c4 * 4], v[c4 * 4 + 1], v[c4 * 4 + 2], v[c4 * 4 + 3]);
-      }
-    }
-    __syncthreads();
+          const float dv = __fadd_rn(x[c], -mean);
+          qs = __fmaf_rn(dv, dv, qs);
+        }
+        red[lr * 4 + lh * 2 + 1] = qs;
+      }
+      wg_barrier(bar);
+#pragma unroll
+      for (int hh = 0; hh < 2; ++hh) {
+        const float4 rs = *reinterpret_cast<const float4*>(red + (fr0 + 8 * hh) * 4);
+        const float mean = __fmul_rn(__fadd_rn(rs.x, rs.z), 1.f / 64.f);
+        const float rstd = 1.f / sqrtf(__fmaf_rn(__fadd_rn(rs.y, rs.w), 1.f / 64.f, 1e-5f));
+#pragma unroll
+        for (int j = 0; j < 8; ++j) {
+          const float2 gj = *reinterpret_cast<const float2*>(&hln[8 * j + fc]);
+          const float2 bj = *reinterpret_cast<const float2*>(&hln[64 + 8 * j + fc]);
+          float& x0 = d[4 * j + 2 * hh];
+          float& x1 = d[4 * j + 2 * hh + 1];
+          x0 = __fmaf_rn(__fmul_rn(__fadd_rn(x0, -mean), rstd), gj.x, bj.x);
+          x1 = __fmaf_rn(__fmul_rn(__fadd_rn(x1, -mean), rstd), gj.y, bj.y);
+        }
+      }
+    }
+#pragma unroll
+    for (int hh = 0; hh < 2; ++hh) {
+      const int row = fr0 + 8 * hh;
+      if (row < nvalid) {
+        float* o = h_out + (long)(node0 + row) * EQD_HID + fc;
+#pragma unroll
+        for (int j = 0; j < 8; ++j) *reinterpret_cast<float2*>(o + 8 * j) = make_float2(d[4 * j + 2 * hh], d[4 * j + 2 * hh + 1]);
+      }
+    }
   }
+  cp_async_wait<0>();
 }
 
 template <int P, bool HLN>
@@ -456,17 +505,19 @@
   if (g->n_nodes <= 0) return EQD_OK;
   eqd::Nm0Consts cst;
   memcpy(&cst, p_l->consts.node, sizeof(cst));
-  int ntiles = (g->n_nodes + EQD_TM - 1) / EQD_TM;
-  size_t smem = sizeof(eqd::Nm0Smem) + 128;
-  int grid = ntiles < EQD_SMS ? ntiles : EQD_SMS;
+  const int ntiles = (g->n_nodes + 63) / 64;
+  int grid = (ntiles + NM_CHAINS - 1) / NM_CHAINS;
+  if (grid > EQD_SMS) grid = EQD_SMS;
   if (hln) {
+    const size_t smem = sizeof(eqd::Nm0Smem) + 128 + NM_HLN_BYTES;
     EQD_SET_SMEM((eqd::node_mlp0_tc_kernel<true>), smem);
-    eqd::node_mlp0_tc_kernel<true><<<grid, NM_THREADS, smem, (cudaStream_t)stream>>>(g->n_nodes, *p, cst, h0, aggr, mu, h_out,
-                                                                                    p_l->norms);
+    eqd::node_mlp0_tc_kernel<true><<<grid, NM_CHAINS * 128, smem, (cudaStream_t)stream>>>(g->n_nodes, *p, cst, h0, aggr,
+                                                                                         mu, h_out, p_l->norms);
   } else {
+    const size_t smem = sizeof(eqd::Nm0Smem) + 128;
     EQD_SET_SMEM((eqd::node_mlp0_tc_kernel<false>), smem);
-    eqd::node_mlp0_tc_kernel<false><<<grid, NM_THREADS, smem, (cudaStream_t)stream>>>(g->n_nodes, *p, cst, h0, aggr, mu,
-                                                                                     h_out, p_l->norms);
+    eqd::node_mlp0_tc_kernel<false><<<grid, NM_CHAINS * 128, smem, (cudaStream_t)stream>>>(g->n_nodes, *p, cst, h0, aggr,
+                                                                                          mu, h_out, p_l->norms);
   }
   EQD_CUDA_LAUNCH_CHECK();
   return EQD_OK;
diff --git a/equidock_public_b200/csrc/proj_tc.cu b/equidock_public_b200/csrc/proj_tc.cu
--- a/equidock_public_b200/csrc/proj_tc.cu
+++ b/equidock_public_b200/csrc/proj_tc.cu
@@ -2,30 +2,10 @@
 
 namespace eqd {
 
-#define PJ_LD 68
-
-template <bool L0>
-struct PjCfg {
-  static constexpr int R = L0 ? 64 : 128;
-  static constexpr int THREADS = 2 * R;
-  static constexpr int KB = L0 ? 5 : 4;
-  static constexpr int GROUP_BYTES = 64 * KB * 16 * 2 * 3;
-  static constexpr int SPLIT_BYTES = 64 * KB * 16 * 2;
-  static constexpr int X_SPLIT_BYTES = 16 * KB * 16 * 2;
-  static constexpr int W_BYTES = 5 * GROUP_BYTES + (L0 ? 3 * X_SPLIT_BYTES : 0);
-  static constexpr int A_SPLIT_BYTES = R * KB * 32;
-  static constexpr int NGROUPS = L0 ? 6 : 5;
-};
+#define PJ_SPLIT_BYTES(KB) (64 * (KB) * 32)
+#define PJ_GROUP_BYTES(KB) (3 * PJ_SPLIT_BYTES(KB))
 
 struct PjConsts { float b[336]; };
-
-template <bool L0>
-struct PjSmem {
-  unsigned char w[PjCfg<L0>::W_BYTES];
-  unsigned char a[3 * PjCfg<L0>::A_SPLIT_BYTES];
-  float d[PjCfg<L0>::R * PJ_LD];
-  unsigned long long w_bar;
-};
 
 __device__ __forceinline__ void store_kv_blocks(unsigned char* __restrict__ kv, long split_stride, int node, int half,
                                                 const float (&v)[32]) {
@@ -41,121 +21,8 @@
   }
 }
 
-template <bool L0>
-__global__ void __launch_bounds__(PjCfg<L0>::THREADS, 1)
-project_tc_kernel(int n_nodes, eqd_layer_params p, const __grid_constant__ PjConsts cst, const float* __restrict__ h, int ldh,
-                  float* __restrict__ proj, int pw, unsigned char* __restrict__ kv, long kv_split_stride, float* __restrict__ x5) {
-  using C = PjCfg<L0>;
-  constexpr int R = C::R;
-  extern __shared__ __align__(128) unsigned char smem_raw[];
-  PjSmem<L0>& S = *reinterpret_cast<PjSmem<L0>*>(smem_raw);
-  const int tid = threadIdx.x, half = tid / R, r = tid % R, warp = tid >> 5, wgi = tid >> 7;
-  const int ntiles = (n_nodes + R - 1) / R;
-  if (tid == 0) {
-    mbar_init(&S.w_bar, 1);
-    asm volatile("fence.mbarrier_init.release.cluster;" ::: "memory");
-    mbar_expect_tx(&S.w_bar, C::W_BYTES);
-    bulk_g2s(S.w, p.w_proj_tc, C::W_BYTES, &S.w_bar);
-  }
-  __syncthreads();
-  const unsigned w_saddr = smem_u32(S.w), a_saddr = smem_u32(S.a);
-  auto a_desc = [&](int s, int kb) { return a_desc_at<R>(a_saddr, C::A_SPLIT_BYTES, wgi, s, kb); };
-  float* dslab = S.d + wgi * 64 * PJ_LD;
-  mbar_wait(&S.w_bar, 0);
-  const float slope = p.leaky_slope;
-  const int lane = tid & 31, wrow0 = (warp * 32) % R;
-
-  for (int tile = blockIdx.x; tile < ntiles; tile += gridDim.x) {
-    const int node0 = tile * R;
-    const int node = node0 + r;
-    const bool valid = node < n_nodes;
-    {
-      float v[32];
-      const float4* hp = reinterpret_cast<const float4*>(h + (long)node * ldh + half * 32);
-#pragma unroll
-      for (int c4 = 0; c4 < 8; ++c4) {
-        float4 t = valid ? hp[c4] : make_float4(0.f, 0.f, 0.f, 0.f);
-        v[c4 * 4] = t.x; v[c4 * 4 + 1] = t.y; v[c4 * 4 + 2] = t.z; v[c4 * 4 + 3] = t.w;
-      }
-      if (L0 && half == 0) {
-        const float4* ep = reinterpret_cast<const float4*>(h + (long)node * ldh + 64);
-        float4 a = valid ? ep[0] : make_float4(0.f, 0.f, 0.f, 0.f), b = valid ? ep[1] : make_float4(0.f, 0.f, 0.f, 0.f);
-        float t[8] = {a.x, a.y, a.z, a.w, b.x, b.y, b.z, b.w};
-        store_extra8_split3<R>(S.a, C::A_SPLIT_BYTES, r, 64, t);
-      }
-      store_half_split3<R>(S.a, C::A_SPLIT_BYTES, r, half * 32, v);
-    }
-    tc_fence_before();
-    __syncthreads();
-#pragma unroll 1
-    for (int grp = 0; grp < C::NGROUPS; ++grp) {
-      if (L0 && grp == 5) {
-        float d[8];
-        wg_gemm6<16>(d, a_desc, [&](int s, int kb) {
-          return b_desc_ex(w_saddr + 5 * C::GROUP_BYTES + s * C::X_SPLIT_BYTES + kb * 512, 256, 128); }, C::KB, false);
-        wg_store_d<16>(dslab, PJ_LD, d, tid & 127);
-        __syncthreads();
-        if (half == 0 && valid) {
-          float e[16];
-#pragma unroll
-          for (int c = 0; c < 16; ++c) {
-            const bool act = (c < 4) || c == 8 || (c >= 10 && c < 15);
-            const float x = S.d[r * PJ_LD + c];
-            e[c] = act ? lrelu(x, slope) : x;
-          }
-          float4* o = reinterpret_cast<float4*>(x5 + (long)node * 16);
-#pragma unroll
-          for (int c4 = 0; c4 < 4; ++c4) o[c4] = make_float4(e[c4 * 4], e[c4 * 4 + 1], e[c4 * 4 + 2], e[c4 * 4 + 3]);
-        }
-        continue;
-      }
-      {
-        float d[32];
-        wg_gemm6<64>(d, a_desc, [&](int s, int kb) {
-          return b_desc_ex(w_saddr + grp * C::GROUP_BYTES + s * C::SPLIT_BYTES + kb * 2048, 1024, 128); }, C::KB, false);
-        wg_store_d<64>(dslab, PJ_LD, d, tid & 127);
-      }
-      __syncthreads();
-      float v[32];
-      tile_ld32f(S.d, PJ_LD, r, half * 32, v);
-      const bool act = (grp == 2 || grp == 3);
-#pragma unroll
-      for (int c = 0; c < 32; ++c) {
-        float t = v[c] + cst.b[grp * 64 + half * 32 + c];
-        v[c] = act ? lrelu(t, slope) : t;
-      }
-      if (grp < 3 || kv == nullptr) {
-        if (L0) {
-          if (valid) {
-            float4* o = reinterpret_cast<float4*>(proj + (long)node * pw + grp * 64 + half * 32);
-#pragma unroll
-            for (int c4 = 0; c4 < 8; ++c4) o[c4] = make_float4(v[c4 * 4], v[c4 * 4 + 1], v[c4 * 4 + 2], v[c4 * 4 + 3]);
-          }
-        } else {
-          float* sc = S.d + r * PJ_LD + half * 32;
-#pragma unroll
-          for (int c4 = 0; c4 < 8; ++c4)
-            *reinterpret_cast<float4*>(sc + c4 * 4) = make_float4(v[c4 * 4], v[c4 * 4 + 1], v[c4 * 4 + 2], v[c4 * 4 + 3]);
-          __syncwarp();
-          float* o = proj + (long)(node0 + wrow0) * pw + grp * 64 + half * 32 + (lane & 7) * 4;
-#pragma unroll
-          for (int i = 0; i < 8; ++i) {
-            const int row = i * 4 + (lane >> 3);
-            float4 t = *reinterpret_cast<const float4*>(S.d + (wrow0 + row) * PJ_LD + half * 32 + (lane & 7) * 4);
-            if (node0 + wrow0 + row < n_nodes) *reinterpret_cast<float4*>(o + (long)row * pw) = t;
-          }
-        }
-      }
-      if (valid && grp >= 3 && kv != nullptr)
-        store_kv_blocks(kv + (long)(grp - 3) * 3 * kv_split_stride, kv_split_stride, node, half, v);
-      __syncthreads();
-    }
-    __syncthreads();
-  }
-}
-
 #define PJ_CHAINS 2
-#define PJ64_W_BYTES (5 * PjCfg<false>::GROUP_BYTES)
+#define PJ64_W_BYTES (5 * PJ_GROUP_BYTES(4))
 #define PJ_OUT_LD 72
 
 struct __align__(128) PjChainSmem {
@@ -204,7 +71,7 @@
     wg_barrier(bar);
     if (tile + tstride < ntiles) stage_h(tile + tstride);
     auto group = [&](int grp) {
-      return [&, grp](int s, int kb) { return b_desc_ex(w_saddr + grp * PjCfg<false>::GROUP_BYTES + s * PjCfg<false>::SPLIT_BYTES + kb * 2048, 1024, 128); };
+      return [&, grp](int s, int kb) { return b_desc_ex(w_saddr + grp * PJ_GROUP_BYTES(4) + s * PJ_SPLIT_BYTES(4) + kb * 2048, 1024, 128); };
     };
     float acc[2][32];
     wg_gemm6_rs_issue<64, 4, 0, false, P>(acc[0], af, group(0), false);
@@ -272,6 +139,136 @@
   cp_async_wait<0>();
 }
 
+#define PJ0_KB 5
+#define PJ0_X_SPLIT_BYTES (16 * PJ0_KB * 32)
+#define PJ0_W_BYTES (5 * PJ_GROUP_BYTES(PJ0_KB) + 3 * PJ0_X_SPLIT_BYTES)
+#define PJ0_PW (128 + 3 * 72)
+
+struct Pj0Smem {
+  unsigned char w[PJ0_W_BYTES];
+  float hs[PJ_CHAINS][64 * 64];
+  float b[320];
+  unsigned long long w_bar;
+};
+
+__global__ void __launch_bounds__(PJ_CHAINS * 128, 1)
+project0_tc_kernel(int n_nodes, eqd_layer_params p, const __grid_constant__ PjConsts cst, const float* __restrict__ h0,
+                   float* __restrict__ proj, unsigned char* __restrict__ kv, long kv_split_stride, float* __restrict__ x5) {
+  extern __shared__ __align__(128) unsigned char smem_raw[];
+  Pj0Smem& S = *reinterpret_cast<Pj0Smem*>(smem_raw);
+  const int tid = threadIdx.x, wgi = tid >> 7, t = tid & 127, lane = t & 31;
+  float* const hs = S.hs[wgi];
+  const int bar = 1 + wgi;
+  const int ntiles = (n_nodes + 63) / 64, tstride = gridDim.x * PJ_CHAINS;
+  if (tid == 0) {
+    mbar_init(&S.w_bar, 1);
+    asm volatile("fence.mbarrier_init.release.cluster;" ::: "memory");
+    mbar_expect_tx(&S.w_bar, PJ0_W_BYTES);
+    bulk_g2s(S.w, p.w_proj_tc, PJ0_W_BYTES, &S.w_bar);
+  }
+  for (int i = tid; i < 320; i += PJ_CHAINS * 128) S.b[i] = cst.b[i];
+  __syncthreads();
+  const unsigned w_saddr = smem_u32(S.w);
+  const float slope = p.leaky_slope;
+  const int fr0 = (t >> 5) * 16 + (lane >> 2), fc = 2 * (lane & 3);
+  auto stage_h = [&](int tile) { stage_rows64(hs, h0, EQD_H0_PAD, 0, (long)tile * 64, min(64, n_nodes - tile * 64), t); };
+  int tile = blockIdx.x * PJ_CHAINS + wgi;
+  if (tile < ntiles) stage_h(tile);
+  mbar_wait(&S.w_bar, 0);
+
+  for (; tile < ntiles; tile += tstride) {
+    const int node0 = tile * 64, nvalid = min(64, n_nodes - node0);
+    unsigned af[3][PJ0_KB][4];
+    extra8_to_a_split3<PJ0_KB>(h0, EQD_H0_PAD, 64, node0, nvalid, t, 4, af);
+    cp_async_wait<0>();
+    wg_barrier(bar);
+    {
+      unsigned a4[3][4][4];
+      staged_rows_to_a_split3(hs, t, a4);
+#pragma unroll
+      for (int sp = 0; sp < 3; ++sp)
+#pragma unroll
+        for (int kb = 0; kb < 4; ++kb)
+#pragma unroll
+          for (int i = 0; i < 4; ++i) af[sp][kb][i] = a4[sp][kb][i];
+    }
+    wg_barrier(bar);
+    if (tile + tstride < ntiles) stage_h(tile + tstride);
+    auto group = [&](int grp) {
+      return [&, grp](int s, int kb) {
+        return b_desc_ex(w_saddr + grp * PJ_GROUP_BYTES(PJ0_KB) + s * PJ_SPLIT_BYTES(PJ0_KB) + kb * 2048, 1024, 128); };
+    };
+    float acc[2][32], d5[8];
+    wg_gemm6_rs_issue<64, PJ0_KB>(acc[0], af, group(0), false);
+#pragma unroll
+    for (int grp = 0; grp < 5; ++grp) {
+      float (&d)[32] = acc[grp & 1];
+      if (grp + 1 < 5)
+        wg_gemm6_rs_issue<64, PJ0_KB>(acc[(grp + 1) & 1], af, group(grp + 1), false);
+      else
+        wg_gemm6_rs_issue<16, PJ0_KB>(d5, af, [&](int s, int kb) {
+          return b_desc_ex(w_saddr + 5 * PJ_GROUP_BYTES(PJ0_KB) + s * PJ0_X_SPLIT_BYTES + kb * 512, 256, 128); }, false);
+      wg_mma_wait<1>(d);
+      const bool act = (grp == 2 || grp == 3);
+#pragma unroll
+      for (int j = 0; j < 8; ++j) {
+        const float2 bj = *reinterpret_cast<const float2*>(&S.b[grp * 64 + 8 * j + fc]);
+#pragma unroll
+        for (int hh = 0; hh < 2; ++hh) {
+          float& x0 = d[4 * j + 2 * hh];
+          float& x1 = d[4 * j + 2 * hh + 1];
+          x0 = x0 + bj.x;
+          x1 = x1 + bj.y;
+          if (act) {
+            x0 = lrelu(x0, slope);
+            x1 = lrelu(x1, slope);
+          }
+        }
+      }
+#pragma unroll
+      for (int hh = 0; hh < 2; ++hh) {
+        const int row = fr0 + 8 * hh, node = node0 + row;
+        if (row >= nvalid) continue;
+        if (grp < 3) {
+          float* o = proj + (long)node * PJ0_PW + grp * 64 + fc;
+#pragma unroll
+          for (int j = 0; j < 8; ++j) *reinterpret_cast<float2*>(o + 8 * j) = make_float2(d[4 * j + 2 * hh], d[4 * j + 2 * hh + 1]);
+        } else {
+          unsigned char* nb = kv + (long)(grp - 3) * 3 * kv_split_stride + (long)(node >> 3) * 1024 + (node & 7) * 16 + fc * 2;
+#pragma unroll
+          for (int j = 0; j < 8; ++j) {
+            unsigned w0, w1, w2;
+            split3_pair(d[4 * j + 2 * hh], d[4 * j + 2 * hh + 1], w0, w1, w2);
+            *reinterpret_cast<unsigned*>(nb + j * 128) = w0;
+            *reinterpret_cast<unsigned*>(nb + kv_split_stride + j * 128) = w1;
+            *reinterpret_cast<unsigned*>(nb + 2 * kv_split_stride + j * 128) = w2;
+          }
+        }
+      }
+    }
+    wg_mma_wait(d5);
+#pragma unroll
+    for (int hh = 0; hh < 2; ++hh) {
+      const int row = fr0 + 8 * hh;
+      if (row >= nvalid) continue;
+      float* o = x5 + (long)(node0 + row) * 16 + fc;
+#pragma unroll
+      for (int j = 0; j < 2; ++j) {
+        float e[2];
+#pragma unroll
+        for (int k = 0; k < 2; ++k) {
+          const int c = 8 * j + fc + k;
+          const bool act = (c < 4) || c == 8 || (c >= 10 && c < 15);
+          const float x = d5[4 * j + 2 * hh + k];
+          e[k] = act ? lrelu(x, slope) : x;
+        }
+        *reinterpret_cast<float2*>(o + 8 * j) = make_float2(e[0], e[1]);
+      }
+    }
+  }
+  cp_async_wait<0>();
+}
+
 __global__ void kv_blocks_kernel(int n_nodes, const float* __restrict__ proj, int pw, int koff, int voff,
                                  unsigned char* __restrict__ kv, long kv_split_stride) {
   int idx = blockIdx.x * blockDim.x + threadIdx.x;
@@ -291,27 +288,6 @@
 
 extern "C" size_t eqd_kv_blocks_bytes(int32_t n_nodes) {
   return (size_t)6 * ((size_t)(n_nodes + 7) / 8 + 8) * 1024;
-}
-
-template <bool L0>
-static int launch_project_tc(const eqd_graph* g, const eqd_layer* p_l, const float* h, int ldh, float* proj, int pw,
-                             void* kv, float* x5, void* stream) {
-  const eqd_layer_params* p = &p_l->dev;
-  if (!(p->leaky_slope >= 0.f && p->leaky_slope <= 1.f)) return EQD_ERR_UNSUPPORTED;
-  if (!p->w_proj_tc || (reinterpret_cast<uintptr_t>(p->w_proj_tc) & 15)) return EQD_ERR_BAD_ARG;
-  if (g->n_nodes <= 0) return EQD_OK;
-  eqd::PjConsts cst;
-  memset(&cst, 0, sizeof(cst));
-  memcpy(&cst, p_l->consts.proj_bias, 320 * sizeof(float));
-  int ntiles = (g->n_nodes + eqd::PjCfg<L0>::R - 1) / eqd::PjCfg<L0>::R;
-  size_t smem = sizeof(eqd::PjSmem<L0>) + 128;
-  EQD_SET_SMEM((eqd::project_tc_kernel<L0>), smem);
-  int grid = ntiles < EQD_SMS ? ntiles : EQD_SMS;
-  long split_stride = (long)((g->n_nodes + 7) / 8 + 8) * 1024;
-  eqd::project_tc_kernel<L0><<<grid, eqd::PjCfg<L0>::THREADS, smem, (cudaStream_t)stream>>>(
-      g->n_nodes, *p, cst, h, ldh, proj, pw, reinterpret_cast<unsigned char*>(kv), split_stride, x5);
-  EQD_CUDA_LAUNCH_CHECK();
-  return EQD_OK;
 }
 
 template <int P>
@@ -351,7 +327,22 @@
   const eqd_layer_params* p = p_l ? &p_l->dev : nullptr;
   if (!g || !p || !h0 || !proj || !kv || !x5) return EQD_ERR_BAD_ARG;
   if (p->dh != 69 || p->dhp != 72 || !eqd_mma_products(p)) return EQD_ERR_UNSUPPORTED;
-  return launch_project_tc<true>(g, p_l, h0, EQD_H0_PAD, proj, 128 + 3 * 72, kv, x5, stream);
+  if (!(p->leaky_slope >= 0.f && p->leaky_slope <= 1.f)) return EQD_ERR_UNSUPPORTED;
+  if (!p->w_proj_tc || (reinterpret_cast<uintptr_t>(p->w_proj_tc) & 15)) return EQD_ERR_BAD_ARG;
+  if (g->n_nodes <= 0) return EQD_OK;
+  eqd::PjConsts cst;
+  memset(&cst, 0, sizeof(cst));
+  memcpy(&cst, p_l->consts.proj_bias, 320 * sizeof(float));
+  const int ntiles = (g->n_nodes + 63) / 64;
+  const size_t smem = sizeof(eqd::Pj0Smem) + 128;
+  EQD_SET_SMEM(eqd::project0_tc_kernel, smem);
+  int grid = (ntiles + PJ_CHAINS - 1) / PJ_CHAINS;
+  if (grid > EQD_SMS) grid = EQD_SMS;
+  const long split_stride = (long)((g->n_nodes + 7) / 8 + 8) * 1024;
+  eqd::project0_tc_kernel<<<grid, PJ_CHAINS * 128, smem, (cudaStream_t)stream>>>(
+      g->n_nodes, *p, cst, h0, proj, reinterpret_cast<unsigned char*>(kv), split_stride, x5);
+  EQD_CUDA_LAUNCH_CHECK();
+  return EQD_OK;
 }
 
 extern "C" int eqd_kv_blocks(const eqd_graph* g, const float* proj, int32_t pw, int32_t koff, int32_t voff, void* kv,
diff --git a/equidock_public_b200/csrc/tc_common.cuh b/equidock_public_b200/csrc/tc_common.cuh
--- a/equidock_public_b200/csrc/tc_common.cuh
+++ b/equidock_public_b200/csrc/tc_common.cuh
@@ -42,16 +42,6 @@
 template <int N, int TB>
 struct Wgmma;
 template <int TB>
-struct Wgmma<16, TB> {
-  static __device__ __forceinline__ void mma(float (&d)[8], unsigned long long a, unsigned long long b, int scale_d) {
-    asm volatile(
-        "{\n\t.reg .pred p;\n\tsetp.ne.b32 p, %10, 0;\n\t"
-        "wgmma.mma_async.sync.aligned.m64n16k16.f32.bf16.bf16 {%0, %1, %2, %3, %4, %5, %6, %7}, %8, %9, p, 1, 1, 0, %11;\n\t}"
-        : "+f"(d[0]), "+f"(d[1]), "+f"(d[2]), "+f"(d[3]), "+f"(d[4]), "+f"(d[5]), "+f"(d[6]), "+f"(d[7])
-        : "l"(a), "l"(b), "r"(scale_d), "n"(TB));
-  }
-};
-template <int TB>
 struct Wgmma<64, TB> {
   static __device__ __forceinline__ void mma(float (&d)[32], unsigned long long a, unsigned long long b, int scale_d) {
     asm volatile(
@@ -61,26 +51,36 @@
         : "l"(a), "l"(b), "r"(scale_d), "n"(TB));
   }
 };
-template <int TB>
-struct Wgmma<80, TB> {
-  static __device__ __forceinline__ void mma(float (&d)[40], unsigned long long a, unsigned long long b, int scale_d) {
-    asm volatile(
-        "{\n\t.reg .pred p;\n\tsetp.ne.b32 p, %42, 0;\n\t"
-        "wgmma.mma_async.sync.aligned.m64n80k16.f32.bf16.bf16 {%0, %1, %2, %3, %4, %5, %6, %7, %8, %9, %10, %11, %12, %13, %14, %15, %16, %17, %18, %19, %20, %21, %22, %23, %24, %25, %26, %27, %28, %29, %30, %31, %32, %33, %34, %35, %36, %37, %38, %39}, %40, %41, p, 1, 1, 0, %43;\n\t}"
-        : "+f"(d[0]), "+f"(d[1]), "+f"(d[2]), "+f"(d[3]), "+f"(d[4]), "+f"(d[5]), "+f"(d[6]), "+f"(d[7]), "+f"(d[8]), "+f"(d[9]), "+f"(d[10]), "+f"(d[11]), "+f"(d[12]), "+f"(d[13]), "+f"(d[14]), "+f"(d[15]), "+f"(d[16]), "+f"(d[17]), "+f"(d[18]), "+f"(d[19]), "+f"(d[20]), "+f"(d[21]), "+f"(d[22]), "+f"(d[23]), "+f"(d[24]), "+f"(d[25]), "+f"(d[26]), "+f"(d[27]), "+f"(d[28]), "+f"(d[29]), "+f"(d[30]), "+f"(d[31]), "+f"(d[32]), "+f"(d[33]), "+f"(d[34]), "+f"(d[35]), "+f"(d[36]), "+f"(d[37]), "+f"(d[38]), "+f"(d[39])
-        : "l"(a), "l"(b), "r"(scale_d), "n"(TB));
-  }
-};
 
 template <int N, int TB>
 struct WgmmaRS;
 template <int TB>
+struct WgmmaRS<16, TB> {
+  static __device__ __forceinline__ void mma(float (&d)[8], const unsigned (&a)[4], unsigned long long b, int scale_d) {
+    asm volatile(
+        "{\n\t.reg .pred p;\n\tsetp.ne.b32 p, %13, 0;\n\t"
+        "wgmma.mma_async.sync.aligned.m64n16k16.f32.bf16.bf16 {%0, %1, %2, %3, %4, %5, %6, %7}, {%8, %9, %10, %11}, %12, p, 1, 1, %14;\n\t}"
+        : "+f"(d[0]), "+f"(d[1]), "+f"(d[2]), "+f"(d[3]), "+f"(d[4]), "+f"(d[5]), "+f"(d[6]), "+f"(d[7])
+        : "r"(a[0]), "r"(a[1]), "r"(a[2]), "r"(a[3]), "l"(b), "r"(scale_d), "n"(TB));
+  }
+};
+template <int TB>
 struct WgmmaRS<64, TB> {
   static __device__ __forceinline__ void mma(float (&d)[32], const unsigned (&a)[4], unsigned long long b, int scale_d) {
     asm volatile(
         "{\n\t.reg .pred p;\n\tsetp.ne.b32 p, %37, 0;\n\t"
         "wgmma.mma_async.sync.aligned.m64n64k16.f32.bf16.bf16 {%0, %1, %2, %3, %4, %5, %6, %7, %8, %9, %10, %11, %12, %13, %14, %15, %16, %17, %18, %19, %20, %21, %22, %23, %24, %25, %26, %27, %28, %29, %30, %31}, {%32, %33, %34, %35}, %36, p, 1, 1, %38;\n\t}"
         : "+f"(d[0]), "+f"(d[1]), "+f"(d[2]), "+f"(d[3]), "+f"(d[4]), "+f"(d[5]), "+f"(d[6]), "+f"(d[7]), "+f"(d[8]), "+f"(d[9]), "+f"(d[10]), "+f"(d[11]), "+f"(d[12]), "+f"(d[13]), "+f"(d[14]), "+f"(d[15]), "+f"(d[16]), "+f"(d[17]), "+f"(d[18]), "+f"(d[19]), "+f"(d[20]), "+f"(d[21]), "+f"(d[22]), "+f"(d[23]), "+f"(d[24]), "+f"(d[25]), "+f"(d[26]), "+f"(d[27]), "+f"(d[28]), "+f"(d[29]), "+f"(d[30]), "+f"(d[31])
+        : "r"(a[0]), "r"(a[1]), "r"(a[2]), "r"(a[3]), "l"(b), "r"(scale_d), "n"(TB));
+  }
+};
+template <int TB>
+struct WgmmaRS<80, TB> {
+  static __device__ __forceinline__ void mma(float (&d)[40], const unsigned (&a)[4], unsigned long long b, int scale_d) {
+    asm volatile(
+        "{\n\t.reg .pred p;\n\tsetp.ne.b32 p, %45, 0;\n\t"
+        "wgmma.mma_async.sync.aligned.m64n80k16.f32.bf16.bf16 {%0, %1, %2, %3, %4, %5, %6, %7, %8, %9, %10, %11, %12, %13, %14, %15, %16, %17, %18, %19, %20, %21, %22, %23, %24, %25, %26, %27, %28, %29, %30, %31, %32, %33, %34, %35, %36, %37, %38, %39}, {%40, %41, %42, %43}, %44, p, 1, 1, %46;\n\t}"
+        : "+f"(d[0]), "+f"(d[1]), "+f"(d[2]), "+f"(d[3]), "+f"(d[4]), "+f"(d[5]), "+f"(d[6]), "+f"(d[7]), "+f"(d[8]), "+f"(d[9]), "+f"(d[10]), "+f"(d[11]), "+f"(d[12]), "+f"(d[13]), "+f"(d[14]), "+f"(d[15]), "+f"(d[16]), "+f"(d[17]), "+f"(d[18]), "+f"(d[19]), "+f"(d[20]), "+f"(d[21]), "+f"(d[22]), "+f"(d[23]), "+f"(d[24]), "+f"(d[25]), "+f"(d[26]), "+f"(d[27]), "+f"(d[28]), "+f"(d[29]), "+f"(d[30]), "+f"(d[31]), "+f"(d[32]), "+f"(d[33]), "+f"(d[34]), "+f"(d[35]), "+f"(d[36]), "+f"(d[37]), "+f"(d[38]), "+f"(d[39])
         : "r"(a[0]), "r"(a[1]), "r"(a[2]), "r"(a[3]), "l"(b), "r"(scale_d), "n"(TB));
   }
 };
@@ -171,16 +171,6 @@
 #pragma unroll
   for (int j = 0; j < 4; ++j) a_store8<R>(a, split_bytes, row, c0 + 8 * j, p0 + 4 * j, p1 + 4 * j, p2 + 4 * j);
 }
-template <int R>
-__device__ __forceinline__ void store_extra8_split3(unsigned char* a, unsigned split_bytes, int row, int c0, const float (&t)[8]) {
-  unsigned p0[8], p1[8], p2[8];
-#pragma unroll
-  for (int c = 0; c < 4; ++c) split3_pair(t[2 * c], t[2 * c + 1], p0[c], p1[c], p2[c]);
-#pragma unroll
-  for (int c = 4; c < 8; ++c) p0[c] = p1[c] = p2[c] = 0u;
-  a_store8<R>(a, split_bytes, row, c0, p0, p1, p2);
-  a_store8<R>(a, split_bytes, row, c0 + 8, p0 + 4, p1 + 4, p2 + 4);
-}
 template <int KB, int P = 6>
 __device__ __forceinline__ void acc_to_a_split3(const float (&v)[8 * KB], unsigned (&a)[3][KB][4]) {
 #pragma unroll
@@ -209,6 +199,19 @@
       const float2 v = *reinterpret_cast<const float2*>(rows + row * 64 + ((k4 ^ stage_swz(row)) << 2) + 2 * (c & 1));
       split3_pair<P>(v.x, v.y, a[0][kb][i], a[1][kb][i], a[2][kb][i]);
     }
+}
+template <int KB, int P = 6>
+__device__ __forceinline__ void extra8_to_a_split3(const float* src, int ld, int c0, long row0, int nvalid, int t, int kb,
+                                                   unsigned (&a)[3][KB][4]) {
+  const int g = (t >> 5) * 16 + ((t & 31) >> 2), fc = 2 * (t & 3);
+#pragma unroll
+  for (int i = 0; i < 2; ++i) {
+    const int row = g + 8 * i;
+    const float2 x = row < nvalid ? *reinterpret_cast<const float2*>(src + (row0 + row) * ld + c0 + fc) : make_float2(0.f, 0.f);
+    split3_pair<P>(x.x, x.y, a[0][kb][i], a[1][kb][i], a[2][kb][i]);
+  }
+#pragma unroll
+  for (int sp = 0; sp < 3; ++sp) a[sp][kb][2] = a[sp][kb][3] = 0u;
 }
 __device__ __forceinline__ void staged_rows_to_frag(const float* rows, int t, float (&v)[32]) {
   const int g = (t >> 5) * 16 + ((t & 31) >> 2), c = t & 3;
```

New measurement: 43720, median of 6. 1.02x the previous value.
